# strasdat/ScaViSLAM

Hardware: AMD Instinct MI355X
Metric: stereo frames/sec + DWO Schur ms @ 50 KF / 20k pts (higher is better)
Workload: dtype u8/int32 (FAST, ZNSSD), f32+f64 (dense tracking), f64 (Schur); 1 GPU

## Files before the change

include/scavislam_hip.h:

```cpp
#ifndef SCAVISLAM_HIP_H
#define SCAVISLAM_HIP_H

#include <stddef.h>
#include <stdint.h>

#ifdef __cplusplus
extern "C" {
#endif

#define SVS_API_VERSION 9
int svs_api_version(void);

enum {
  SVS_OK = 0,
  SVS_ERR_INVALID = 1,
  SVS_ERR_HIP = 2,
  SVS_ERR_NO_DEVICE = 3,
  SVS_ERR_CAPACITY = 4,
  SVS_ERR_UNSUPPORTED = 5,
  SVS_ERR_BUSY = 6
};

#define SVS_NUM_PYR_LEVELS 3
#define SVS_MAX_CELLS 64

typedef struct { double f, cx, cy, b; int32_t w, h; } svs_cam;

typedef struct {
  int32_t gx, gy, cell_w, cell_h;
  int32_t min_inner, min_outer, max_inner, max_outer;
  int32_t fast_min, fast_max;
  int32_t thr[SVS_MAX_CELLS];
} svs_fastgrid;

typedef struct {
  double xyz_anchor[3];
  double anchor_obs_pyr[3];
  int32_t anchor_level, kf_index, point_id, pad_;
} svs_candidate_point;

typedef struct {
  double T_anchor_from_w[12];
  const uint8_t *pyr[3];
  int32_t stride[3];
  int32_t pad_;
} svs_keyframe;

enum { SVS_MATCH_OK = 0, SVS_MATCH_NO_ANCHOR, SVS_MATCH_BORDER, SVS_MATCH_DEPTH,
       SVS_MATCH_TEXTURE, SVS_MATCH_NONE, SVS_MATCH_NO_DISP,
       SVS_MATCH_SKIPPED  };

typedef struct {
  int32_t status, u, v, znssd;
  double obs[3];
  double xyz_actkey[3];
} svs_match_result;

typedef struct {
  double H[21];
  double b[6];
  double chi2;
  int64_t n_valid;
} svs_dense_sums;

typedef struct {
  double obs[3];
  double info[3];
  int32_t point, pose, anchor, pad_;
} svs_ba_edge;

typedef struct {
  double T_21[12];
  double info[36];
  int32_t pose1, pose2;
} svs_ba_constraint;

typedef struct {
  int32_t num_iters;
  int32_t use_robust;
  double huber_delta;
  double lambda_init;
  int32_t max_trials;
  int32_t self_edge_mode;
} svs_ba_params;

typedef struct {
  int32_t iterations, trials, accepted, terminated;
  double chi2_init, chi2_final, lambda_final;
} svs_ba_stats;

typedef struct svs_ctx svs_ctx;
int svs_ctx_create(int device, void *hip_stream, svs_ctx **out);
int svs_ctx_destroy(svs_ctx *ctx);
int svs_ctx_sync(svs_ctx *ctx);
int svs_ctx_set_option(svs_ctx *ctx, const char *name, int value);
int svs_ctx_get_stat(svs_ctx *ctx, const char *name, long long *out);
void *svs_ctx_stream(svs_ctx *ctx);
const char *svs_last_error(svs_ctx *ctx);
int svs_malloc(svs_ctx *ctx, size_t bytes, void **d_ptr);
int svs_free(svs_ctx *ctx, void *d_ptr);
int svs_memcpy_h2d(svs_ctx *ctx, void *d_dst, const void *h_src, size_t bytes);
int svs_memcpy_d2h(svs_ctx *ctx, void *h_dst, const void *d_src, size_t bytes);
int svs_timer_start(svs_ctx *ctx);
int svs_timer_stop_ms(svs_ctx *ctx, float *ms);

int svs_pyr_down_u8(svs_ctx *ctx, const uint8_t *d_src, int w, int h, int sstride, size_t s_bstride,
                    uint8_t *d_dst, int dstride, size_t d_bstride, int batch);
int svs_convert_sobel_f32(svs_ctx *ctx, const uint8_t *d_src, int w, int h, int sstride,
                          size_t s_bstride, float *d_img, float *d_dx, float *d_dy, int fstride,
                          size_t f_bstride, int batch);

typedef struct {
  int32_t prefilter_cap;
  int32_t sad_window;
  int32_t min_disparity;
  int32_t num_disparities;
  int32_t texture_threshold;
  int32_t uniqueness_ratio;
  int32_t speckle_window;
  int32_t speckle_range;
  int32_t disp12_max_diff;
} svs_stereo_params;
typedef struct svs_stereo svs_stereo;
int svs_stereo_create(svs_ctx *ctx, int w, int h, int max_batch, const svs_stereo_params *prm, svs_stereo **out);
int svs_stereo_destroy(svs_stereo *s);
int svs_stereo_compute(svs_stereo *s, const uint8_t *d_left, int lstride, size_t l_bstride, const uint8_t *d_right,
                       int rstride, size_t r_bstride, float *d_disp, int dstride, size_t d_bstride, int n_batch);

typedef struct svs_fast svs_fast;
int svs_fast_create(svs_ctx *ctx, int n_levels, const int32_t *w, const int32_t *h,
                    const svs_fastgrid *grids, int batch, int corner_cap_per_level,
                    svs_fast **out);
int svs_fast_destroy(svs_fast *f);
int svs_fast_detect(svs_fast *f, const uint8_t *const *d_img, const int32_t *stride,
                    const size_t *bstride, int n_batch, int trials);
int svs_fast_download(svs_fast *f, int slot, int level, int16_t *h_xy, int cap, int32_t *h_n,
                      int32_t *h_cell_count, int32_t *h_emit_thr, int32_t *h_thr_state);
int svs_fast_set_thresholds(svs_fast *f, int slot, int level, const int32_t *h_thr);
int svs_fast_device_view(svs_fast *f, int level, const uint32_t **d_corner_bits, int32_t *row_stride_bytes, size_t *batch_stride_bytes,
                         int32_t *cell_column_bits, const int32_t **d_emit_thr, size_t *emit_bstride);

typedef struct {
  const svs_keyframe *d_kfs; int32_t n_kf;
  const svs_candidate_point *d_pts; int32_t n_pts;
  const double *d_T_cur_from_w;
  const double *d_T_w_from_actkey;
  const uint8_t *d_cur_pyr[3]; int32_t cur_stride[3]; size_t cur_bstride[3];
  const float *d_disp; int32_t disp_stride; size_t disp_bstride;
  svs_cam cam_vec[3];
  int32_t search_radius, thr_mean, thr_std;
  int32_t n_batch;
  size_t kf_bstride, pts_bstride, out_bstride;
} svs_match_args;
int svs_match(svs_ctx *ctx, const svs_match_args *a, svs_fast *f, svs_match_result *d_out);

typedef struct {
  int32_t robust_kernel;
  int32_t num_iter;
  double kernel_param;
  double initial_mu;
  double tau;
  int32_t min_obs;
  int32_t pad_;
} svs_pose_opt_params;
void svs_pose_opt_params_default(svs_pose_opt_params *p);
typedef struct {
  double initial_chi2, chi2, max_err;
  int32_t num_obs;
  int32_t status;
} svs_pose_opt_stats;
int svs_motion_only(svs_ctx *ctx, const svs_match_result *d_results, int n, size_t res_bstride, const svs_cam *cam,
                    const svs_pose_opt_params *prm, double *d_T_io, svs_pose_opt_stats *d_stats, int batch);

typedef struct {
  int32_t accepted;
  int32_t is_new;
  double uv_pyr[2];
  double curkey_uv_pyr[2];
} svs_gated_point;
typedef struct {
  int32_t num_points_grid2x2[4];
  int32_t num_points_grid3x3[9];
  int32_t num_matched_points[3];
  int32_t num_track_points;
  int32_t num_obs;
  int32_t pad_[2];
  double sum_track_length;
} svs_point_stats;
int svs_process_matched_points(svs_ctx *ctx, const svs_match_result *d_results, const svs_candidate_point *d_pts, int n,
                               size_t res_bstride, size_t pts_bstride, int n_new_records, const svs_cam *cam,
                               const double *d_T, float max_reproj_error, svs_gated_point *d_gated, size_t gated_bstride,
                               svs_point_stats *d_stats, int batch);

int svs_pointcloud_cpu_sem(svs_ctx *ctx, const float *d_disp, int disp_stride, size_t disp_bstride,
                           const svs_cam *cam, int level, const double *d_T_cur_from_actkey,
                           float *d_cloud, size_t cloud_bstride, int batch);
int svs_dense_pass_cpu_sem(svs_ctx *ctx, const float *d_cloud, size_t cloud_bstride,
                           const uint8_t *d_prev_u8, int pstride, size_t p_bstride,
                           const float *d_cur, const float *d_dx, const float *d_dy, int fstride,
                           size_t f_bstride, const svs_cam *cam, const double *d_T, int do_jac,
                           svs_dense_sums *d_out, int batch);
typedef struct {
  int32_t level;
  int32_t accepted;
  float chi2, new_chi2;
} svs_dense_lm_record;
typedef struct {
  const float *d_cloud[3]; size_t cloud_bstride[3];
  const uint8_t *d_prev_u8[3]; int32_t pstride[3]; size_t p_bstride[3];
  const float *d_cur[3]; const float *d_dx[3]; const float *d_dy[3];
  int32_t fstride[3]; size_t f_bstride[3];
  svs_cam cam_vec[3];
  const uint8_t *d_cur_u8[3]; int32_t c8stride[3]; size_t c8_bstride[3];
  double *d_T_jac_out;
  svs_dense_lm_record *d_record_out;
  int32_t record_cap;
  int32_t *d_n_record_out;
} svs_dense_track_args;
int svs_dense_track_cpu_sem(svs_ctx *ctx, const svs_dense_track_args *a, double *d_T_io,
                            int32_t *d_passes_out, int batch);
int svs_dense_seq_sum_f32(svs_ctx *ctx, const float *d_terms, int n, size_t bstride, int batch, int how, float *d_out, int32_t *d_fell_back);
int svs_dense_residual_image_cpu_sem(svs_ctx *ctx, const float *d_cloud, size_t cloud_bstride,
                                     const uint8_t *d_prev_u8, int pstride, size_t p_bstride,
                                     const float *d_cur, int fstride, size_t f_bstride,
                                     const uint8_t *d_cur_u8, int c8stride, size_t c8_bstride,
                                     const svs_cam *cam, const double *d_T, size_t T_bstride,
                                     float *d_res_img4, size_t res_bstride, int batch);
int svs_preprocess_gpu_sem(svs_ctx *ctx, const uint8_t *d_src, int w, int h, int sstride, size_t s_bstride,
                           float *const *d_img, float *const *d_dx, float *const *d_dy, const int32_t *fstride,
                           const size_t *f_bstride, int levels, int batch);
typedef struct {
  const float *d_cloud4[3]; int32_t stride_f4[3]; size_t cloud_bstride[3];
  const float *d_prev[3];
  const float *d_cur[3];
  const float *d_dx[3], *d_dy[3];
  int32_t stride_f[3]; size_t f_bstride[3];
  int32_t w[3], h[3];
  double f[3], cx[3], cy[3];
  double *d_T_jac_out;
  svs_dense_lm_record *d_record_out;
  int32_t record_cap;
  int32_t *d_n_record_out;
} svs_dense_track_full_args;
int svs_dense_track_full(svs_ctx *ctx, const svs_dense_track_full_args *a, double *d_T_io, int32_t *d_passes_out, int batch);
int svs_dense_pixel_terms_full(svs_ctx *ctx, const float *d_cloud4, int w, int h, int stride_f4, const float *d_prev,
                               const float *d_cur, const float *d_dx, const float *d_dy, int stride_f, float f, float cx,
                               float cy, const float *h_T34_colmajor, float *d_terms8);
int svs_dense_pass_full(svs_ctx *ctx, const float *d_cloud4, int w, int h, int stride_f4,
                        const float *d_prev, const float *d_cur, const float *d_dx,
                        const float *d_dy, int stride_f, float f, float cx, float cy,
                        const float *h_T34_colmajor, int do_jac, svs_dense_sums *d_out);
int svs_dense_residual_image_full(svs_ctx *ctx, const float *d_cloud4, int w, int h, int stride_f4,
                                  const float *d_prev, const float *d_cur, int stride_f, float f,
                                  float cx, float cy, const float *h_T34_colmajor, float *d_res_img4);
int svs_pointcloud_full(svs_ctx *ctx, const float *h_TQ_colmajor, const float *d_disp, int w, int h,
                        int stride_in, int stride_out, int factor, float *d_cloud4);
int svs_pointcloud_full_pose(svs_ctx *ctx, const double *d_T, const svs_cam *cam, const float *d_disp, int disp_stride, size_t disp_bstride,
                             int w, int h, int stride_out, size_t cloud_bstride, int factor, float *d_cloud4, int batch);

typedef struct {
  int32_t fast_trials;
  int32_t search_radius, thr_mean, thr_std;
  float max_reproj_error;
  int32_t use_block_matching;
  svs_pose_opt_params pose_opt;
  svs_stereo_params stereo;
  int32_t n_levels;
  int32_t num_max_points;
  int32_t min_matches;
  int32_t cuda_build;
} svs_frontend_params;
typedef struct {
  double T_cur_from_actkey[12];
  int32_t dense_passes;
  int32_t n_points;
  int32_t n_matched;
  int32_t tracking_ok;
  svs_pose_opt_stats pose_stats;
  svs_point_stats point_stats;
} svs_frame_result;
typedef struct svs_frontend svs_frontend;
int svs_frontend_create(svs_ctx *ctx, const svs_cam *cam, const svs_frontend_params *prm, int max_points, int max_keyframes, svs_frontend **out);
int svs_frontend_create_batch(svs_ctx *ctx, const svs_cam *cam, const svs_frontend_params *prm, int max_points, int max_keyframes, int n_streams,
                              svs_frontend **out);
int svs_frontend_destroy(svs_frontend *fe);
int svs_frontend_first_frame(svs_frontend *fe, const uint8_t *h_left, int lstride, const uint8_t *h_right, int rstride, const float *h_disp, int dstride);
int svs_frontend_keep_keyframe(svs_frontend *fe, int slot, const double *T_kf_from_w);
int svs_frontend_keep_keyframe_of(svs_frontend *fe, int stream, int slot, const double *T_kf_from_w);
int svs_frontend_keep_keyframes(svs_frontend *fe, int slot, const double *h_T_kf_from_w);
int svs_frontend_set_candidates(svs_frontend *fe, const svs_candidate_point *h_pts, int n, int n_new_records);
int svs_frontend_set_candidates_grouped(svs_frontend *fe, int stream, const svs_candidate_point *h_pts, int n, const int32_t *h_group_end, int n_groups);
int svs_frontend_set_candidates_all(svs_frontend *fe, const svs_candidate_point *h_pts, const int32_t *h_n, const int32_t *h_group_end, int n_groups);
int svs_frontend_process_frame(svs_frontend *fe, const uint8_t *h_left, int lstride, const uint8_t *h_right, int rstride, const float *h_disp,
                               int dstride, const double *T_cur_from_actkey, const double *T_actkey_from_w, svs_frame_result *out,
                               svs_match_result *h_matches, svs_gated_point *h_gated);
int svs_frontend_submit_frame(svs_frontend *fe, const uint8_t *h_left, int lstride, const uint8_t *h_right, int rstride, const float *h_disp, int dstride,
                              const double *T_cur_from_actkey, const double *T_actkey_from_w, int want_matches, int want_gated);
int svs_frontend_wait_frame(svs_frontend *fe, svs_frame_result *out, svs_match_result *h_matches, svs_gated_point *h_gated);
int svs_frontend_prefetch_frame(svs_frontend *fe, const uint8_t *h_left, int lstride, const uint8_t *h_right, int rstride, const float *h_disp, int dstride);
int svs_frontend_staging_view(svs_frontend *fe, uint8_t **h_left, uint8_t **h_right, float **h_disp);
typedef struct {
  const uint8_t *d_left; int32_t lstride; size_t l_bstride;
  const uint8_t *d_right; int32_t rstride; size_t r_bstride;
  const float *d_disp; int32_t dstride; size_t d_bstride;
  void *ready_event;
} svs_frames_dev;
int svs_frontend_input_view(svs_frontend *fe, uint8_t **d_left, int32_t *lstride, size_t *l_bstride, uint8_t **d_right, int32_t *rstride, size_t *r_bstride,
                            float **d_disp, int32_t *dstride, size_t *d_bstride);
int svs_frontend_first_frames(svs_frontend *fe, const svs_frames_dev *in);
int svs_frontend_process_frames(svs_frontend *fe, const svs_frames_dev *in, const double *h_T_cur_from_actkey, const double *h_T_actkey_from_w);
int svs_frontend_results(svs_frontend *fe, int stream, svs_frame_result *out, svs_match_result *h_matches, svs_gated_point *h_gated);
int svs_frontend_poses(svs_frontend *fe, double *h_T_cur_from_actkey, int32_t *h_tracking_ok);
#define SVS_FRONTEND_STAGES 8
int svs_frontend_set_timing(svs_frontend *fe, int on);
int svs_frontend_stage_times(svs_frontend *fe, float *ms);
int svs_frontend_dense_records(svs_frontend *fe, int stream, svs_dense_lm_record *h_rec, int cap, int32_t *n);
int svs_frontend_recompute_cloud(svs_frontend *fe, const double *T_cur_from_actkey);
int svs_frontend_device_view(svs_frontend *fe, int stream, const uint8_t **d_pyr_last, int32_t *stride, const float **d_disp, const float **d_cloud,
                             svs_fast **fast);

typedef struct {
  int32_t clearance;
  int32_t num_max_points;
  int32_t min_num_points;
  int32_t n_levels;
} svs_seed_params;
void svs_seed_params_default(svs_seed_params *p);
typedef struct {
  double T_newkey_from_cur[12];
  uint64_t seed;
  int32_t add_flags[9];
  int32_t n0[3];
  int32_t n_tree;
  int32_t kf_index, first_point_id;
  int32_t use_order;
  int32_t n_order[3];
  int32_t pad_;
} svs_seed_problem;
typedef struct {
  const int16_t *d_xy[3]; size_t xy_bstride[3]; int32_t xy_cap[3];
  const int32_t *d_n[3]; size_t n_bstride[3];
  const int32_t *d_cell_count[3]; size_t cell_bstride[3]; int32_t n_cells[3];
  const float *d_disp; int32_t disp_stride; size_t disp_bstride;
  svs_cam cam;
  const svs_seed_problem *d_prob;
  const double *d_tree_xy; const int32_t *d_tree_level; size_t tree_bstride;
  const int32_t *d_order[3]; size_t order_bstride[3];
  int32_t batch;
} svs_seed_args;
int svs_seed_points(svs_ctx *ctx, const svs_seed_args *a, const svs_seed_params *prm, svs_candidate_point *d_out, int cap, int32_t *d_n_new);
enum { SVS_SEED_FIRST = 0,
       SVS_SEED_MORE = 1 };
typedef struct {
  int32_t stream, mode;
  int32_t kf_index, first_point_id;
  double T_newkey_from_cur[12];
  uint64_t seed;
  const int32_t *h_order[3];
  int32_t n_order[3];
  int32_t pad_;
} svs_seed_request;
int svs_frontend_seed_keyframes(svs_frontend *fe, int n, const svs_seed_request *req, const svs_seed_params *prm, svs_candidate_point *h_out, int cap_per_request,
                                int32_t *h_n_new);

int svs_rectify_build_maps(const double *K, const double *dist, const double *R, const double *Knew, int w, int h, int16_t *map_xy, uint16_t *map_frac);
typedef struct svs_rectify svs_rectify;
int svs_rectify_create(svs_ctx *ctx, int w, int h, int max_batch, const int16_t *h_left_xy, const uint16_t *h_left_frac, const int16_t *h_right_xy,
                       const uint16_t *h_right_frac, svs_rectify **out);
int svs_rectify_destroy(svs_rectify *r);
typedef struct {
  const uint8_t *d_left; int32_t lstride; size_t l_bstride;
  int32_t left_channels;
  const uint8_t *d_right; int32_t rstride; size_t r_bstride;
  void *ready_event;
} svs_raw_frames_dev;
int svs_rectify_frames(svs_rectify *r, const svs_raw_frames_dev *raw, uint8_t *d_left_out, int lstride, size_t l_bstride, uint8_t *d_right_out, int rstride,
                       size_t r_bstride, int n_batch);
int svs_depth_to_disp(svs_ctx *ctx, const svs_cam *cam, const uint16_t *d_depth16, int stride, size_t bstride, float *d_disp, int dstride, size_t d_bstride,
                      int n_batch);

typedef struct svs_loop svs_loop;
int svs_loop_create(svs_ctx *ctx, const svs_cam *cam, int desc_dim, int max_desc, int max_places, int max_hyp, int max_checks, svs_loop **out);
int svs_loop_destroy(svs_loop *l);
int svs_loop_set_place(svs_loop *l, int slot, int n, const float *h_desc, const double *h_uvu, const double *h_xyz);
typedef struct {
  int32_t query_slot, train_slot;
  int32_t n_hyp;
  double pixel_thr;
  uint64_t seed;
  const int32_t *h_samples;
} svs_loop_check;
typedef struct {
  int32_t n_matches;
  int32_t n_inliers;
  int32_t best_hyp;
  int32_t n_invalid_hyp;
  double T_query_from_train[12];
} svs_loop_result;
int svs_loop_check_batch(svs_loop *l, int n_checks, const svs_loop_check *checks, svs_loop_result *h_results, int32_t *h_train_idx, float *h_distance,
                         uint8_t *h_inlier, int32_t *h_samples_out, int32_t *h_hyp_inliers);
int svs_loop_set_timing(svs_loop *l, int on);
int svs_loop_stage_times(svs_loop *l, float *ms);

#define SVS_LOOP_MAX_WORDS 1048576
int svs_loop_set_vocabulary(svs_loop *l, int n_words, const float *h_words);
typedef struct {
  int32_t slot;
  int32_t do_loop_detection;
  const int32_t *h_exclude;
  int32_t n_exclude;
  float radius;
  float min_score;
} svs_loop_location;
typedef struct {
  int32_t number_of_words;
  int32_t n_scored;
  int32_t best_slot;
  float best_score;
  int32_t candidate;
} svs_loop_location_result;
int svs_loop_add_locations(svs_loop *l, int n, const svs_loop_location *locs, svs_loop_location_result *h_results, int32_t *h_word, float *h_word_d2,
                           float *h_scores);
int svs_loop_index_stage_times(svs_loop *l, float *ms);

#define SVS_VOCAB_MAX_POINTS 2097152
typedef struct {
  int32_t n_words;
  int32_t iterations;
  uint64_t seed;
  const float *h_init;
  int32_t drop_empty;
} svs_vocab_params;
typedef struct {
  int32_t n_words_out, n_seeded, iterations_run, converged, n_empty;
  uint64_t inertia_q28;
} svs_vocab_result;
void svs_vocab_params_default(svs_vocab_params *p);
int svs_vocab_train(svs_ctx *ctx, int desc_dim, int n, const float *h_desc, const svs_vocab_params *prm, float *h_words, svs_vocab_result *h_res,
                    int32_t *h_seed_index, int32_t *h_assign, float *h_assign_d2, int32_t *h_count, int32_t *h_changed);
int svs_vocab_stage_times(svs_ctx *ctx, float *ms);

typedef struct svs_surf svs_surf;
typedef struct {
  float hessian_threshold;
  int32_t n_octaves, n_octave_layers;
  int32_t require_disparity;
} svs_surf_params;
typedef struct { float x, y, size, angle, response; int32_t octave, laplacian, pad_; } svs_surf_keypoint;
#define SVS_SURF_STAGES 6
void svs_surf_params_default(svs_surf_params *p);
int svs_surf_create(svs_ctx *ctx, const svs_cam *cam, int w, int h, int max_batch, int max_keypoints, const svs_surf_params *prm, svs_surf **out);
int svs_surf_destroy(svs_surf *s);
int svs_surf_extract(svs_surf *s, const uint8_t *d_img, int stride, size_t bstride, const float *d_disp, int dstride, size_t d_bstride, int n_batch,
                     int32_t *h_count, int32_t *h_overflow, svs_surf_keypoint *h_kp, double *h_uvu, float *h_desc);
int svs_loop_set_place_from_surf(svs_loop *l, int slot, svs_surf *s, int image_index);
int svs_surf_set_timing(svs_surf *s, int on);
int svs_surf_stage_times(svs_surf *s, float *ms);

enum { SVS_REG_LOCAL = 0, SVS_REG_LOOP = 1 };
enum { SVS_REG_OK = 0, SVS_REG_FEW_CANDIDATES = 1, SVS_REG_FEW_MATCHES_PASS1 = 2, SVS_REG_FEW_MATCHES_PASS2 = 3, SVS_REG_NOT_COVISIBLE = 4 };
enum { SVS_REG_KF_IN_WINDOW = 1,
       SVS_REG_KF_DIRECT_NEIGHBOR = 2 };
typedef struct {
  int32_t covis_thr;
  int32_t search_radius[2];
  int32_t thr_mean, thr_std;
  int32_t num_iter[2];
  int32_t pad_;
  double reproj_thr;
  double kernel_param;
} svs_reg_params;
void svs_reg_params_default(svs_reg_params *p);
typedef struct {
  int32_t mode;
  int32_t n_kf, n_src;
  int32_t root_kf;
  const float *d_root_disp;
  int32_t root_disp_stride, pad_;
  int32_t fast_thr[SVS_NUM_PYR_LEVELS][SVS_MAX_CELLS];
  double T_root_from_world[12];
  const svs_keyframe *h_kfs;
  const uint8_t *h_kf_flags;
  const svs_candidate_point *h_src;
  const int32_t *h_obs_begin;
  const int32_t *h_obs_kf;
} svs_reg_request;
typedef struct {
  int32_t status;
  int32_t n_candidates, n_obs_pass1, n_obs_pass2, n_accepted;
  int32_t n_qualified;
  double T_newroot_from_oldroot[12];
  double T_pass1[12];
  svs_pose_opt_stats stats_pass1, stats_pass2;
} svs_reg_result;
typedef struct {
  int32_t strength;
  int32_t n_u_hi, n_u_lo, n_v_hi, n_v_lo;
  int32_t qualifies;
  int32_t in_vertex_table;
  int32_t pad_;
} svs_reg_kf_stats;
typedef struct svs_reg svs_reg;
int svs_reg_create(svs_ctx *ctx, const svs_cam *cam, int max_requests, int max_points, int max_keyframes, int max_observers, svs_reg **out);
int svs_reg_destroy(svs_reg *reg);
int svs_reg_register_batch(svs_reg *reg, int n_requests, const svs_reg_request *req, const svs_reg_params *prm, svs_reg_result *h_res, int32_t *h_cand_src,
                           svs_match_result *h_matches, int32_t *h_status_pass1, int32_t *h_accepted, svs_reg_kf_stats *h_kf_stats,
                           svs_match_result *h_matches_pass1);
#define SVS_REG_STAGES 7
int svs_reg_set_timing(svs_reg *reg, int on);
int svs_reg_stage_times(svs_reg *reg, float *ms);

typedef struct { char bytes[128]; } svs_unique_id;
typedef struct svs_comm svs_comm;
int svs_comm_get_unique_id(svs_ctx *ctx, svs_unique_id *out);
int svs_comm_create(svs_ctx *ctx, const svs_unique_id *id, int rank, int world, svs_comm **out);
int svs_comm_destroy(svs_comm *c);
int svs_comm_allreduce_f64(svs_comm *c, void *d_buf, size_t count);
int svs_comm_stats(svs_comm *c, int32_t *rank, int32_t *world, uint64_t *n_calls, uint64_t *n_doubles);
typedef struct { char bytes[64]; } svs_ipc_handle;
int svs_comm_create_p2p(svs_ctx *ctx, int rank, int world, size_t capacity_doubles, svs_comm **out, svs_ipc_handle *h_mine);
int svs_comm_connect_p2p(svs_comm *c, const svs_ipc_handle *h_all);
int svs_comm_transport(svs_comm *c, int32_t *kind, uint32_t *timeouts);

typedef struct svs_ba svs_ba;
typedef int (*svs_allreduce_fn)(void *d_buf, size_t count, void *user);

int svs_ba_create(svs_ctx *ctx, svs_ba **out);
int svs_ba_destroy(svs_ba *ba);
int svs_ba_set_problem(svs_ba *ba, int P, const double *h_poses, int L, const double *h_psi,
                       int E, const svs_ba_edge *h_edges, int C, const svs_ba_constraint *h_cons,
                       const svs_cam *cam, const svs_ba_params *prm, int add_pose_terms);
int svs_ba_window_update(svs_ba *ba, int P, const int32_t *h_pose_ids, const double *h_poses, int L, const int32_t *h_point_ids,
                         const double *h_psi, const int32_t *h_anchor_pose_ids, int n_new, const svs_ba_edge *h_new_obs, int C,
                         const svs_ba_constraint *h_cons, const svs_cam *cam, const svs_ba_params *prm);
int svs_ba_window_reset(svs_ba *ba);
int svs_ba_window_forget_keyframes(svs_ba *ba, const int32_t *h_pose_ids, int n);
int svs_ba_optimize(svs_ba *ba, svs_allreduce_fn allreduce, void *user, svs_ba_stats *stats);
int svs_ba_optimize_batch(svs_ba *const *bas, int n, svs_ba_stats *stats);
int svs_ba_get_state(svs_ba *ba, double *h_poses, double *h_psi);
int svs_ba_set_comm(svs_ba *ba, svs_comm *comm);
int svs_ba_set_option(svs_ba *ba, const char *name, int value);
int svs_ba_reset_state(svs_ba *ba, const double *h_poses, const double *h_psi);
int svs_ba_reduced_system(svs_ba *ba, double lambda, double *h_Hred ,
                          double *h_bred , double *h_chi2);
int svs_ba_schur_layout(svs_ba *ba, int32_t *waves_per_workgroup, int32_t *big_pool);
int svs_ba_trial(svs_ba *ba, double lambda, const double *h_xp, double *h_poses_trial, double *h_psi_trial, double *h_chi2_trial,
                 double *h_scale_l);
int svs_ba_info(svs_ba *ba, int32_t *solve_kind, int32_t *envelope_rows, int32_t *n_chunks, int32_t *n_wide);
int svs_ba_order_info(svs_ba *ba, int32_t *ordered, int32_t *envelope_rows_caller_order, int32_t *h_perm);
int svs_ba_set_timing(svs_ba *ba, int on);
int svs_ba_kernel_times(svs_ba *ba, float *reduce_ms, float *solve_ms, float *backsub_ms,
                        int32_t *n_reduce_launches);
int svs_ba_graph_stats(svs_ba *ba, int64_t *launches, int64_t *captures);

#ifdef __cplusplus
}
#endif
#endif
```

scavislam_amd/capi.py:

```python
import ctypes as C
import os
import weakref

from .ctypes_types import BaParams, BaStats, Cam, FastGrid, LoopCheck, LoopLocation, LoopLocationResult, LoopResult, PoseOptParams, PoseOptStats, RegParams, RegRequest, RegResult, SeedArgs, SeedParams, SeedRequest, StereoParams, SurfParams, VocabParams, VocabResult

_HERE = os.path.dirname(os.path.abspath(__file__))
LIB_PATH = os.environ.get("SVS_LIB_PATH") or os.path.join(_HERE, "libscavislam_hip.so")
_LIB = None

ALLREDUCE_FN = C.CFUNCTYPE(C.c_int, C.c_void_p, C.c_size_t, C.c_void_p)


class SvsError(RuntimeError):
    pass


class DenseTrackArgs(C.Structure):
    _fields_ = [("d_cloud", C.c_void_p * 3), ("cloud_bstride", C.c_size_t * 3),
                ("d_prev_u8", C.c_void_p * 3), ("pstride", C.c_int32 * 3), ("p_bstride", C.c_size_t * 3),
                ("d_cur", C.c_void_p * 3), ("d_dx", C.c_void_p * 3), ("d_dy", C.c_void_p * 3),
                ("fstride", C.c_int32 * 3), ("f_bstride", C.c_size_t * 3), ("cam_vec", Cam * 3),
                ("d_cur_u8", C.c_void_p * 3), ("c8stride", C.c_int32 * 3), ("c8_bstride", C.c_size_t * 3),
                ("d_T_jac_out", C.c_void_p), ("d_record_out", C.c_void_p), ("record_cap", C.c_int32), ("d_n_record_out", C.c_void_p)]


class DenseTrackFullArgs(C.Structure):
    _fields_ = [("d_cloud4", C.c_void_p * 3), ("stride_f4", C.c_int32 * 3), ("cloud_bstride", C.c_size_t * 3),
                ("d_prev", C.c_void_p * 3), ("d_cur", C.c_void_p * 3), ("d_dx", C.c_void_p * 3), ("d_dy", C.c_void_p * 3),
                ("stride_f", C.c_int32 * 3), ("f_bstride", C.c_size_t * 3),
                ("w", C.c_int32 * 3), ("h", C.c_int32 * 3),
                ("f", C.c_double * 3), ("cx", C.c_double * 3), ("cy", C.c_double * 3),
                ("d_T_jac_out", C.c_void_p), ("d_record_out", C.c_void_p), ("record_cap", C.c_int32),
                ("d_n_record_out", C.c_void_p)]


class FrontendParams(C.Structure):
    _fields_ = [("fast_trials", C.c_int32), ("search_radius", C.c_int32), ("thr_mean", C.c_int32), ("thr_std", C.c_int32),
                ("max_reproj_error", C.c_float), ("use_block_matching", C.c_int32), ("pose_opt", PoseOptParams), ("stereo", StereoParams),
                ("n_levels", C.c_int32), ("num_max_points", C.c_int32), ("min_matches", C.c_int32), ("cuda_build", C.c_int32)]

    @classmethod
    def reference(cls, use_block_matching=False, cuda_build=False, n_levels=3, search_radius=None, thr_mean=22, thr_std=10, num_max_points=300):
        if search_radius is None:
            search_radius = 4 if cuda_build else 8
        return cls(6, search_radius, thr_mean, thr_std, 2.0, int(use_block_matching), PoseOptParams.reference(), StereoParams.reference(),
                   n_levels, num_max_points, 20, int(cuda_build))


class FramesDev(C.Structure):
    _fields_ = [("d_left", C.c_void_p), ("lstride", C.c_int32), ("l_bstride", C.c_size_t),
                ("d_right", C.c_void_p), ("rstride", C.c_int32), ("r_bstride", C.c_size_t),
                ("d_disp", C.c_void_p), ("dstride", C.c_int32), ("d_bstride", C.c_size_t),
                ("ready_event", C.c_void_p)]


class PointStatsC(C.Structure):
    _fields_ = [("num_points_grid2x2", C.c_int32 * 4), ("num_points_grid3x3", C.c_int32 * 9), ("num_matched_points", C.c_int32 * 3),
                ("num_track_points", C.c_int32), ("num_obs", C.c_int32), ("pad_", C.c_int32 * 2), ("sum_track_length", C.c_double)]


class FrameResult(C.Structure):
    _fields_ = [("T_cur_from_actkey", C.c_double * 12), ("dense_passes", C.c_int32), ("n_points", C.c_int32), ("n_matched", C.c_int32),
                ("tracking_ok", C.c_int32), ("pose_stats", PoseOptStats), ("point_stats", PointStatsC)]


class MatchArgs(C.Structure):
    _fields_ = [("d_kfs", C.c_void_p), ("n_kf", C.c_int32),
                ("d_pts", C.c_void_p), ("n_pts", C.c_int32),
                ("d_T_cur_from_w", C.c_void_p), ("d_T_w_from_actkey", C.c_void_p),
                ("d_cur_pyr", C.c_void_p * 3), ("cur_stride", C.c_int32 * 3), ("cur_bstride", C.c_size_t * 3),
                ("d_disp", C.c_void_p), ("disp_stride", C.c_int32), ("disp_bstride", C.c_size_t),
                ("cam_vec", Cam * 3),
                ("search_radius", C.c_int32), ("thr_mean", C.c_int32), ("thr_std", C.c_int32),
                ("n_batch", C.c_int32),
                ("kf_bstride", C.c_size_t), ("pts_bstride", C.c_size_t), ("out_bstride", C.c_size_t)]


class RawFramesDev(C.Structure):
    _fields_ = [("d_left", C.c_void_p), ("lstride", C.c_int32), ("l_bstride", C.c_size_t), ("left_channels", C.c_int32),
                ("d_right", C.c_void_p), ("rstride", C.c_int32), ("r_bstride", C.c_size_t),
                ("ready_event", C.c_void_p)]


_SIGS = {
    "svs_ctx_create": [C.c_int, C.c_void_p, C.POINTER(C.c_void_p)],
    "svs_ctx_destroy": [C.c_void_p],
    "svs_ctx_sync": [C.c_void_p],
    "svs_ctx_set_option": [C.c_void_p, C.c_char_p, C.c_int],
    "svs_ctx_get_stat": [C.c_void_p, C.c_char_p, C.POINTER(C.c_longlong)],
    "svs_malloc": [C.c_void_p, C.c_size_t, C.POINTER(C.c_void_p)],
    "svs_free": [C.c_void_p, C.c_void_p],
    "svs_memcpy_h2d": [C.c_void_p, C.c_void_p, C.c_void_p, C.c_size_t],
    "svs_memcpy_d2h": [C.c_void_p, C.c_void_p, C.c_void_p, C.c_size_t],
    "svs_timer_start": [C.c_void_p],
    "svs_timer_stop_ms": [C.c_void_p, C.POINTER(C.c_float)],
    "svs_pyr_down_u8": [C.c_void_p, C.c_void_p, C.c_int, C.c_int, C.c_int, C.c_size_t, C.c_void_p, C.c_int,
                        C.c_size_t, C.c_int],
    "svs_convert_sobel_f32": [C.c_void_p, C.c_void_p, C.c_int, C.c_int, C.c_int, C.c_size_t, C.c_void_p,
                              C.c_void_p, C.c_void_p, C.c_int, C.c_size_t, C.c_int],
    "svs_fast_create": [C.c_void_p, C.c_int, C.POINTER(C.c_int32), C.POINTER(C.c_int32), C.POINTER(FastGrid),
                        C.c_int, C.c_int, C.POINTER(C.c_void_p)],
    "svs_fast_destroy": [C.c_void_p],
    "svs_fast_detect": [C.c_void_p, C.POINTER(C.c_void_p), C.POINTER(C.c_int32), C.POINTER(C.c_size_t),
                        C.c_int, C.c_int],
    "svs_fast_download": [C.c_void_p, C.c_int, C.c_int, C.c_void_p, C.c_int, C.POINTER(C.c_int32),
                          C.c_void_p, C.c_void_p, C.c_void_p],
    "svs_fast_set_thresholds": [C.c_void_p, C.c_int, C.c_int, C.c_void_p],
    "svs_fast_device_view": [C.c_void_p, C.c_int, C.POINTER(C.c_void_p), C.POINTER(C.c_int32), C.POINTER(C.c_size_t), C.POINTER(C.c_int32),
                             C.POINTER(C.c_void_p), C.POINTER(C.c_size_t)],
    "svs_match": [C.c_void_p, C.POINTER(MatchArgs), C.c_void_p, C.c_void_p],
    "svs_pointcloud_cpu_sem": [C.c_void_p, C.c_void_p, C.c_int, C.c_size_t, C.POINTER(Cam), C.c_int,
                               C.c_void_p, C.c_void_p, C.c_size_t, C.c_int],
    "svs_dense_pass_cpu_sem": [C.c_void_p, C.c_void_p, C.c_size_t, C.c_void_p, C.c_int, C.c_size_t,
                               C.c_void_p, C.c_void_p, C.c_void_p, C.c_int, C.c_size_t, C.POINTER(Cam),
                               C.c_void_p, C.c_int, C.c_void_p, C.c_int],
    "svs_dense_seq_sum_f32": [C.c_void_p, C.c_void_p, C.c_int, C.c_size_t, C.c_int, C.c_int, C.c_void_p, C.c_void_p],
    "svs_dense_track_cpu_sem": [C.c_void_p, C.POINTER(DenseTrackArgs), C.c_void_p, C.c_void_p, C.c_int],
    "svs_dense_residual_image_cpu_sem": [C.c_void_p, C.c_void_p, C.c_size_t, C.c_void_p, C.c_int, C.c_size_t,
                                         C.c_void_p, C.c_int, C.c_size_t, C.c_void_p, C.c_int, C.c_size_t,
                                         C.POINTER(Cam), C.c_void_p, C.c_size_t, C.c_void_p, C.c_size_t, C.c_int],
    "svs_dense_residual_image_full": [C.c_void_p, C.c_void_p, C.c_int, C.c_int, C.c_int, C.c_void_p, C.c_void_p,
                                      C.c_int, C.c_float, C.c_float, C.c_float, C.c_void_p, C.c_void_p],
    "svs_preprocess_gpu_sem": [C.c_void_p, C.c_void_p, C.c_int, C.c_int, C.c_int, C.c_size_t, C.POINTER(C.c_void_p), C.POINTER(C.c_void_p),
                               C.POINTER(C.c_void_p), C.POINTER(C.c_int32), C.POINTER(C.c_size_t), C.c_int, C.c_int],
    "svs_dense_track_full": [C.c_void_p, C.POINTER(DenseTrackFullArgs), C.c_void_p, C.c_void_p, C.c_int],
    "svs_dense_pixel_terms_full": [C.c_void_p, C.c_void_p, C.c_int, C.c_int, C.c_int, C.c_void_p, C.c_void_p, C.c_void_p, C.c_void_p,
                                   C.c_int, C.c_float, C.c_float, C.c_float, C.c_void_p, C.c_void_p],
    "svs_dense_pass_full": [C.c_void_p, C.c_void_p, C.c_int, C.c_int, C.c_int, C.c_void_p, C.c_void_p,
                            C.c_void_p, C.c_void_p, C.c_int, C.c_float, C.c_float, C.c_float, C.c_void_p,
                            C.c_int, C.c_void_p],
    "svs_pointcloud_full": [C.c_void_p, C.c_void_p, C.c_void_p, C.c_int, C.c_int, C.c_int, C.c_int, C.c_int,
                            C.c_void_p],
    "svs_motion_only": [C.c_void_p, C.c_void_p, C.c_int, C.c_size_t, C.POINTER(Cam), C.POINTER(PoseOptParams), C.c_void_p, C.c_void_p,
                        C.c_int],
    "svs_process_matched_points": [C.c_void_p, C.c_void_p, C.c_void_p, C.c_int, C.c_size_t, C.c_size_t, C.c_int, C.POINTER(Cam),
                                   C.c_void_p, C.c_float, C.c_void_p, C.c_size_t, C.c_void_p, C.c_int],
    "svs_stereo_create": [C.c_void_p, C.c_int, C.c_int, C.c_int, C.POINTER(StereoParams), C.POINTER(C.c_void_p)],
    "svs_stereo_destroy": [C.c_void_p],
    "svs_stereo_compute": [C.c_void_p, C.c_void_p, C.c_int, C.c_size_t, C.c_void_p, C.c_int, C.c_size_t, C.c_void_p, C.c_int,
                           C.c_size_t, C.c_int],
    "svs_frontend_create": [C.c_void_p, C.POINTER(Cam), C.POINTER(FrontendParams), C.c_int, C.c_int, C.POINTER(C.c_void_p)],
    "svs_frontend_create_batch": [C.c_void_p, C.POINTER(Cam), C.POINTER(FrontendParams), C.c_int, C.c_int, C.c_int, C.POINTER(C.c_void_p)],
    "svs_frontend_keep_keyframe_of": [C.c_void_p, C.c_int, C.c_int, C.c_void_p],
    "svs_frontend_set_candidates_grouped": [C.c_void_p, C.c_int, C.c_void_p, C.c_int, C.c_void_p, C.c_int],
    "svs_frontend_keep_keyframes": [C.c_void_p, C.c_int, C.c_void_p],
    "svs_frontend_set_candidates_all": [C.c_void_p, C.c_void_p, C.c_void_p, C.c_void_p, C.c_int],
    "svs_frontend_submit_frame": [C.c_void_p, C.c_void_p, C.c_int, C.c_void_p, C.c_int, C.c_void_p, C.c_int, C.c_void_p, C.c_void_p, C.c_int, C.c_int],
    "svs_frontend_wait_frame": [C.c_void_p, C.POINTER(FrameResult), C.c_void_p, C.c_void_p],
    "svs_frontend_prefetch_frame": [C.c_void_p, C.c_void_p, C.c_int, C.c_void_p, C.c_int, C.c_void_p, C.c_int],
    "svs_frontend_staging_view": [C.c_void_p, C.POINTER(C.c_void_p), C.POINTER(C.c_void_p), C.POINTER(C.c_void_p)],
    "svs_frontend_input_view": [C.c_void_p, C.POINTER(C.c_void_p), C.POINTER(C.c_int32), C.POINTER(C.c_size_t), C.POINTER(C.c_void_p), C.POINTER(C.c_int32),
                                C.POINTER(C.c_size_t), C.POINTER(C.c_void_p), C.POINTER(C.c_int32), C.POINTER(C.c_size_t)],
    "svs_frontend_first_frames": [C.c_void_p, C.POINTER(FramesDev)],
    "svs_frontend_process_frames": [C.c_void_p, C.POINTER(FramesDev), C.c_void_p, C.c_void_p],
    "svs_frontend_results": [C.c_void_p, C.c_int, C.POINTER(FrameResult), C.c_void_p, C.c_void_p],
    "svs_frontend_poses": [C.c_void_p, C.c_void_p, C.c_void_p],
    "svs_frontend_set_timing": [C.c_void_p, C.c_int],
    "svs_frontend_stage_times": [C.c_void_p, C.c_void_p],
    "svs_frontend_dense_records": [C.c_void_p, C.c_int, C.c_void_p, C.c_int, C.POINTER(C.c_int32)],
    "svs_pointcloud_full_pose": [C.c_void_p, C.c_void_p, C.POINTER(Cam), C.c_void_p, C.c_int, C.c_size_t, C.c_int, C.c_int, C.c_int, C.c_size_t, C.c_int,
                                 C.c_void_p, C.c_int],
    "svs_frontend_destroy": [C.c_void_p],
    "svs_frontend_first_frame": [C.c_void_p, C.c_void_p, C.c_int, C.c_void_p, C.c_int, C.c_void_p, C.c_int],
    "svs_frontend_keep_keyframe": [C.c_void_p, C.c_int, C.c_void_p],
    "svs_frontend_set_candidates": [C.c_void_p, C.c_void_p, C.c_int, C.c_int],
    "svs_frontend_process_frame": [C.c_void_p, C.c_void_p, C.c_int, C.c_void_p, C.c_int, C.c_void_p, C.c_int, C.c_void_p, C.c_void_p,
                                   C.POINTER(FrameResult), C.c_void_p, C.c_void_p],
    "svs_frontend_recompute_cloud": [C.c_void_p, C.c_void_p],
    "svs_frontend_device_view": [C.c_void_p, C.c_int, C.c_void_p, C.c_void_p, C.c_void_p, C.c_void_p, C.c_void_p],
    "svs_rectify_build_maps": [C.c_void_p, C.c_void_p, C.c_void_p, C.c_void_p, C.c_int, C.c_int, C.c_void_p, C.c_void_p],
    "svs_rectify_create": [C.c_void_p, C.c_int, C.c_int, C.c_int, C.c_void_p, C.c_void_p, C.c_void_p, C.c_void_p, C.POINTER(C.c_void_p)],
    "svs_rectify_destroy": [C.c_void_p],
    "svs_rectify_frames": [C.c_void_p, C.POINTER(RawFramesDev), C.c_void_p, C.c_int, C.c_size_t, C.c_void_p, C.c_int, C.c_size_t, C.c_int],
    "svs_depth_to_disp": [C.c_void_p, C.POINTER(Cam), C.c_void_p, C.c_int, C.c_size_t, C.c_void_p, C.c_int, C.c_size_t, C.c_int],
    "svs_seed_points": [C.c_void_p, C.POINTER(SeedArgs), C.POINTER(SeedParams), C.c_void_p, C.c_int, C.c_void_p],
    "svs_frontend_seed_keyframes": [C.c_void_p, C.c_int, C.POINTER(SeedRequest), C.POINTER(SeedParams), C.c_void_p, C.c_int, C.c_void_p],
    "svs_loop_create": [C.c_void_p, C.POINTER(Cam), C.c_int, C.c_int, C.c_int, C.c_int, C.c_int, C.POINTER(C.c_void_p)],
    "svs_loop_destroy": [C.c_void_p],
    "svs_loop_set_place": [C.c_void_p, C.c_int, C.c_int, C.c_void_p, C.c_void_p, C.c_void_p],
    "svs_loop_check_batch": [C.c_void_p, C.c_int, C.POINTER(LoopCheck), C.POINTER(LoopResult), C.c_void_p, C.c_void_p, C.c_void_p, C.c_void_p, C.c_void_p],
    "svs_loop_set_timing": [C.c_void_p, C.c_int],
    "svs_loop_stage_times": [C.c_void_p, C.c_void_p],
    "svs_loop_set_vocabulary": [C.c_void_p, C.c_int, C.c_void_p],
    "svs_loop_add_locations": [C.c_void_p, C.c_int, C.POINTER(LoopLocation), C.POINTER(LoopLocationResult), C.c_void_p, C.c_void_p, C.c_void_p],
    "svs_loop_index_stage_times": [C.c_void_p, C.c_void_p],
    "svs_vocab_train": [C.c_void_p, C.c_int, C.c_int, C.c_void_p, C.POINTER(VocabParams), C.c_void_p, C.POINTER(VocabResult), C.c_void_p, C.c_void_p, C.c_void_p,
                        C.c_void_p, C.c_void_p],
    "svs_vocab_stage_times": [C.c_void_p, C.c_void_p],
    "svs_surf_create": [C.c_void_p, C.POINTER(Cam), C.c_int, C.c_int, C.c_int, C.c_int, C.POINTER(SurfParams), C.POINTER(C.c_void_p)],
    "svs_surf_destroy": [C.c_void_p],
    "svs_surf_extract": [C.c_void_p, C.c_void_p, C.c_int, C.c_size_t, C.c_void_p, C.c_int, C.c_size_t, C.c_int, C.c_void_p, C.c_void_p, C.c_void_p, C.c_void_p,
                         C.c_void_p],
    "svs_loop_set_place_from_surf": [C.c_void_p, C.c_int, C.c_void_p, C.c_int],
    "svs_surf_set_timing": [C.c_void_p, C.c_int],
    "svs_surf_stage_times": [C.c_void_p, C.c_void_p],
    "svs_reg_create": [C.c_void_p, C.POINTER(Cam), C.c_int, C.c_int, C.c_int, C.c_int, C.POINTER(C.c_void_p)],
    "svs_reg_destroy": [C.c_void_p],
    "svs_reg_register_batch": [C.c_void_p, C.c_int, C.POINTER(RegRequest), C.POINTER(RegParams), C.POINTER(RegResult), C.c_void_p, C.c_void_p, C.c_void_p, C.c_void_p,
                               C.c_void_p, C.c_void_p],
    "svs_reg_set_timing": [C.c_void_p, C.c_int],
    "svs_reg_stage_times": [C.c_void_p, C.c_void_p],
    "svs_ba_create": [C.c_void_p, C.POINTER(C.c_void_p)],
    "svs_ba_destroy": [C.c_void_p],
    "svs_ba_set_problem": [C.c_void_p, C.c_int, C.c_void_p, C.c_int, C.c_void_p, C.c_int, C.c_void_p,
                           C.c_int, C.c_void_p, C.POINTER(Cam), C.POINTER(BaParams), C.c_int],
    "svs_ba_window_update": [C.c_void_p, C.c_int, C.c_void_p, C.c_void_p, C.c_int, C.c_void_p, C.c_void_p, C.c_void_p, C.c_int, C.c_void_p, C.c_int,
                             C.c_void_p, C.POINTER(Cam), C.POINTER(BaParams)],
    "svs_ba_window_reset": [C.c_void_p],
    "svs_ba_window_forget_keyframes": [C.c_void_p, C.c_void_p, C.c_int],
    "svs_ba_optimize": [C.c_void_p, C.c_void_p, C.c_void_p, C.POINTER(BaStats)],
    "svs_ba_optimize_batch": [C.POINTER(C.c_void_p), C.c_int, C.POINTER(BaStats)],
    "svs_ba_get_state": [C.c_void_p, C.c_void_p, C.c_void_p],
    "svs_ba_reset_state": [C.c_void_p, C.c_void_p, C.c_void_p],
    "svs_ba_reduced_system": [C.c_void_p, C.c_double, C.c_void_p, C.c_void_p, C.c_void_p],
    "svs_ba_info": [C.c_void_p, C.POINTER(C.c_int32), C.POINTER(C.c_int32), C.POINTER(C.c_int32), C.POINTER(C.c_int32)],
    "svs_ba_schur_layout": [C.c_void_p, C.POINTER(C.c_int32), C.POINTER(C.c_int32)],
    "svs_ba_trial": [C.c_void_p, C.c_double, C.c_void_p, C.c_void_p, C.c_void_p, C.c_void_p, C.c_void_p],
    "svs_ba_order_info": [C.c_void_p, C.POINTER(C.c_int32), C.POINTER(C.c_int32), C.c_void_p],
    "svs_ba_set_timing": [C.c_void_p, C.c_int],
    "svs_ba_set_option": [C.c_void_p, C.c_char_p, C.c_int],
    "svs_ba_set_comm": [C.c_void_p, C.c_void_p],
    "svs_comm_get_unique_id": [C.c_void_p, C.c_void_p],
    "svs_comm_create": [C.c_void_p, C.c_void_p, C.c_int, C.c_int, C.POINTER(C.c_void_p)],
    "svs_comm_destroy": [C.c_void_p],
    "svs_comm_allreduce_f64": [C.c_void_p, C.c_void_p, C.c_size_t],
    "svs_comm_stats": [C.c_void_p, C.POINTER(C.c_int32), C.POINTER(C.c_int32), C.POINTER(C.c_uint64), C.POINTER(C.c_uint64)],
    "svs_comm_create_p2p": [C.c_void_p, C.c_int, C.c_int, C.c_size_t, C.POINTER(C.c_void_p), C.c_void_p],
    "svs_comm_connect_p2p": [C.c_void_p, C.c_void_p],
    "svs_comm_transport": [C.c_void_p, C.POINTER(C.c_int32), C.POINTER(C.c_uint32)],
    "svs_ba_kernel_times": [C.c_void_p, C.POINTER(C.c_float), C.POINTER(C.c_float), C.POINTER(C.c_float),
                            C.POINTER(C.c_int32)],
    "svs_ba_graph_stats": [C.c_void_p, C.POINTER(C.c_int64), C.POINTER(C.c_int64)],
}
EXPORTS = sorted(list(_SIGS) + ["svs_ctx_stream", "svs_last_error", "svs_api_version", "svs_pose_opt_params_default", "svs_seed_params_default", "svs_reg_params_default", "svs_vocab_params_default", "svs_surf_params_default"])
API_VERSION = 9


def load():
    global _LIB
    if _LIB is None:
        if not os.path.exists(LIB_PATH):
            raise SvsError(f"{LIB_PATH} not built: run `python -c 'import __graft_entry__ as g; g.build()'` "
                           "(there is no CPU fallback)")
        import torch
        lib = C.CDLL(LIB_PATH)
        for name, args in _SIGS.items():
            fn = getattr(lib, name)
            fn.argtypes = args
            fn.restype = C.c_int
        lib.svs_ctx_stream.argtypes = [C.c_void_p]
        lib.svs_ctx_stream.restype = C.c_void_p
        lib.svs_last_error.argtypes = [C.c_void_p]
        lib.svs_last_error.restype = C.c_char_p
        lib.svs_api_version.argtypes = []
        lib.svs_api_version.restype = C.c_int
        lib.svs_pose_opt_params_default.argtypes = [C.c_void_p]
        lib.svs_pose_opt_params_default.restype = None
        lib.svs_seed_params_default.argtypes = [C.c_void_p]
        lib.svs_seed_params_default.restype = None
        lib.svs_reg_params_default.argtypes = [C.c_void_p]
        lib.svs_reg_params_default.restype = None
        lib.svs_vocab_params_default.argtypes = [C.c_void_p]
        lib.svs_vocab_params_default.restype = None
        lib.svs_surf_params_default.argtypes = [C.c_void_p]
        lib.svs_surf_params_default.restype = None
        if lib.svs_api_version() != API_VERSION:
            raise SvsError(f"{LIB_PATH} was built with SVS_API_VERSION {lib.svs_api_version()}, this binding expects {API_VERSION}: rebuild (__graft_entry__.build())")
        _LIB = lib
    return _LIB


class Context:

    def __init__(self, device=0, stream_ptr=None):
        self.lib = load()
        h = C.c_void_p()
        rc = self.lib.svs_ctx_create(int(device), C.c_void_p(stream_ptr) if stream_ptr else None, C.byref(h))
        if rc:
            raise SvsError(f"svs_ctx_create failed with status {rc} (no gfx950 device visible?)")
        self.h = h
        self.device = device
        self.children = weakref.WeakSet()

    def check(self, rc):
        if rc:
            raise SvsError(f"status {rc}: {self.lib.svs_last_error(self.h).decode(errors='replace')}")

    def call(self, name, *args):
        self.check(getattr(self.lib, name)(self.h, *args))

    def sync(self):
        self.check(self.lib.svs_ctx_sync(self.h))

    def set_option(self, name, value):
        self.call("svs_ctx_set_option", name.encode(), int(value))

    def get_stat(self, name):
        v = C.c_longlong(0)
        self.call("svs_ctx_get_stat", name.encode(), C.byref(v))
        return int(v.value)

    def timer_start(self):
        self.check(self.lib.svs_timer_start(self.h))

    def timer_stop_ms(self):
        ms = C.c_float()
        self.check(self.lib.svs_timer_stop_ms(self.h, C.byref(ms)))
        return ms.value

    def close(self):
        if self.h:
            for ch in list(self.children):
                ch.close()
            self.lib.svs_ctx_destroy(self.h)
            self.h = None

    def __del__(self):
        try:
            self.close()
        except Exception:
            pass


def torch_context(device=0):
    import torch
    torch.cuda.set_device(device)
    s = torch.cuda.Stream(device=device)
    return Context(device, s.cuda_stream), s
```

scavislam_amd/csrc/dense.hip:

```cpp
#include "common.h"
#include "lm6.h"
#include "seqsum.h"
#include <algorithm>
#include <climits>

namespace {

constexpr int NSUM = 28;

struct Acc {
  double v[NSUM];
  int n;
  __device__ __forceinline__ void zero() {
#pragma unroll
    for (int i = 0; i < NSUM; ++i) v[i] = 0;
    n = 0;
  }
};

template <class P>
__device__ __forceinline__ float interp32f(P m, int stride, float u, float v) {
  float x = floorf(u), y = floorf(v);
  float sx = u - x, sy = v - y;
  float wx0 = 1 - sx, wx1 = sx, wy0 = 1 - sy, wy1 = sy;
  int xi = (int)x, yi = (int)y;
  const P p = m + (unsigned)(yi * stride + xi);
  float v00 = p[0], v10 = p[1], v01 = p[stride], v11 = p[stride + 1];
  return (wx0 * wy0) * v00 + (wx0 * wy1) * v01 + (wx1 * wy0) * v10 + (wx1 * wy1) * v11;
}

struct LevelArgs {
  const float *cloud; const uint8_t *prev; const float *cur, *dx, *dy;
  int pstride, fstride;
  svs_cam cam;
  const uint8_t *cur8;
  int c8stride;
};

#define SVS_AS1 __attribute__((address_space(1)))
typedef float svs_f4 __attribute__((ext_vector_type(4)));
struct LevelArgsG {
  const SVS_AS1 float *cloud; const SVS_AS1 uint8_t *prev; const SVS_AS1 float *cur, *dx, *dy;
  int pstride, fstride;
  svs_cam cam;
  const SVS_AS1 uint8_t *cur8;
  int c8stride;
};
__device__ __forceinline__ float4 load_f4(const float *p) { return *reinterpret_cast<const float4 *>(p); }
__device__ __forceinline__ float4 load_f4(const SVS_AS1 float *p) { const svs_f4 v = *(const SVS_AS1 svs_f4 *)p; return make_float4(v.x, v.y, v.z, v.w); }
__device__ __forceinline__ uint32_t load_u32_unaligned(const uint8_t *p) { uint32_t w; __builtin_memcpy(&w, p, 4); return w; }
__device__ __forceinline__ uint32_t load_u32_unaligned(const SVS_AS1 uint8_t *p) {
  typedef uint32_t u32_unaligned __attribute__((aligned(1)));
  return *(const SVS_AS1 u32_unaligned *)p;
}

struct TapRows { uint32_t w[4]; };
constexpr bool TRK_TAPS_ASM = true;
template <bool ASM, class P>
__device__ __forceinline__ void taps_u8_issue(P img, int stride, float u, float v, TapRows &t) {
  const int xi = (int)floorf(u), yi = (int)floorf(v);
  const unsigned o0 = __umul24(yi - 1, stride) + (unsigned)(xi - 1);
  __builtin_amdgcn_sched_barrier(0);
  if constexpr (ASM) {
    const unsigned long long bv = (unsigned long long)img;
    const unsigned long long b0 = ((unsigned long long)(unsigned)__builtin_amdgcn_readfirstlane((int)(bv >> 32)) << 32) | (unsigned)__builtin_amdgcn_readfirstlane((int)bv);
    const unsigned long long rs = (unsigned long long)(unsigned)__builtin_amdgcn_readfirstlane(stride);
    asm("global_load_dword %0, %4, %5\n\t"
        "global_load_dword %1, %4, %6\n\t"
        "global_load_dword %2, %4, %7\n\t"
        "global_load_dword %3, %4, %8"
        : "=&v"(t.w[0]), "=&v"(t.w[1]), "=&v"(t.w[2]), "=&v"(t.w[3])
        : "v"(o0), "s"(b0), "s"(b0 + rs), "s"(b0 + 2 * rs), "s"(b0 + 3 * rs));
  } else {
#pragma unroll
    for (int r = 0; r < 4; ++r) t.w[r] = load_u32_unaligned(img + (o0 + (unsigned)(r * stride)));
  }
  __builtin_amdgcn_sched_barrier(0);
}
template <bool ASM>
__device__ __forceinline__ void taps_u8_wait(TapRows &t) {
  __builtin_amdgcn_sched_barrier(0);
  if constexpr (ASM) {
    asm("s_waitcnt vmcnt(0)" : "+v"(t.w[0]), "+v"(t.w[1]), "+v"(t.w[2]), "+v"(t.w[3]));
    __builtin_amdgcn_sched_barrier(0);
  }
}
__device__ __forceinline__ void taps_u8_finish(const TapRows &t, float u, float v, float &ic, float &gx, float &gy) {
  const float sc = (float)(1. / 255.);
  const float x = floorf(u), y = floorf(v);
  const float sx = u - x, sy = v - y;
  const float wx0 = 1 - sx, wx1 = sx, wy0 = 1 - sy, wy1 = sy;
  float f[4][4];
#pragma unroll
  for (int r = 0; r < 4; ++r)
#pragma unroll
    for (int c = 0; c < 4; ++c) f[r][c] = (float)((t.w[r] >> (8 * c)) & 0xff) * sc;
  const float w00 = wx0 * wy0, w01 = wx0 * wy1, w10 = wx1 * wy0, w11 = wx1 * wy1;
  ic = w00 * f[1][1] + w01 * f[2][1] + w10 * f[1][2] + w11 * f[2][2];
  gx = w00 * (f[1][2] - f[1][0]) + w01 * (f[2][2] - f[2][0]) + w10 * (f[1][3] - f[1][1]) + w11 * (f[2][3] - f[2][1]);
  gy = w00 * (f[2][1] - f[0][1]) + w01 * (f[3][1] - f[1][1]) + w10 * (f[2][2] - f[0][2]) + w11 * (f[3][2] - f[1][2]);
}
template <class P>
__device__ __forceinline__ void taps_u8(P img, int stride, float u, float v, float &ic, float &gx, float &gy) {
  TapRows t;
  taps_u8_issue<false>(img, stride, u, v, t);
  taps_u8_finish(t, u, v, ic, gx, gy);
}

struct SampleIn { float4 c4; uint8_t prev; };
template <class LA>
__device__ __forceinline__ SampleIn sample_load(const LA &L, int u, int v, int cw, bool in_range) {
  SampleIn s;
  s.c4 = in_range ? load_f4(L.cloud + 4u * (__umul24(v, cw) + (unsigned)u)) : make_float4(0.f, 0.f, 1.f, -1.f);
  s.prev = L.prev[__umul24((in_range ? v : 0) * 4, L.pstride) + (unsigned)((in_range ? u : 0) * 4)];
  return s;
}
__device__ __forceinline__ double rcp_rn(double b) {
  double r = __builtin_amdgcn_rcp(b);
  double e = __builtin_fma(-b, r, 1.0);
  r = __builtin_fma(e, r, r);
  e = __builtin_fma(-b, r, 1.0);
  return __builtin_fma(e, r, r);
}
__device__ __forceinline__ double div_rn(double a, double b, double r) {
  const double q = a * r;
  return __builtin_fma(__builtin_fma(-q, b, a), r, q);
}

template <bool JAC, bool U8SRC = false, int TM = 0, class LA = LevelArgs>
__device__ __forceinline__ void sample_cpu_sem(const LA &L, const double *T, const SampleIn &in, bool in_range, Acc &a,
                                               const float *ip_lut = nullptr, float *term_out = nullptr) {
  const float4 c4 = in.c4;
  bool ok = in_range && (c4.w > 0);
  const double xp0 = c4.x, xp1 = c4.y, xp2 = c4.z;
  const double x = T[0] * xp0 + T[1] * xp1 + T[2] * xp2 + T[3];
  const double y = T[4] * xp0 + T[5] * xp1 + T[6] * xp2 + T[7];
  const double z = T[8] * xp0 + T[9] * xp1 + T[10] * xp2 + T[11];
  const double rz = rcp_rn(z);
  float uvx = (float)(L.cam.f * div_rn(x, z, rz) + L.cam.cx);
  float uvy = (float)(L.cam.f * div_rn(y, z, rz) + L.cam.cy);
  ok = ok && (fabsf(uvx) < 1e9f && fabsf(uvy) < 1e9f);
  const int ui = ok ? (int)uvx : 0, vi = ok ? (int)uvy : 0;
  ok = ok && (ui >= 2 && vi >= 2 && ui < L.cam.w - 2 && vi < L.cam.h - 2);
  if (!ok) { uvx = 2.f; uvy = 2.f; }
  const float ip = ip_lut ? ip_lut[in.prev] : (float)((1. / 255.) * in.prev);
  TapRows taps;
  if constexpr (U8SRC) taps_u8_issue<TRK_TAPS_ASM>(L.cur8, L.c8stride, uvx, uvy, taps);
  const double zs = ok ? z : 1.0, xs = ok ? x : 0.0, ys = ok ? y : 0.0;
  const double f = L.cam.f, iz = ok ? rz : 1.0, iz2 = iz * iz, fx = f * iz, xz = xs * iz2 * f, yz = ys * iz2 * f;
  float ic, g8x = 0.f, g8y = 0.f;
  if constexpr (U8SRC) { taps_u8_wait<TRK_TAPS_ASM>(taps); taps_u8_finish(taps, uvx, uvy, ic, g8x, g8y); }
  else ic = interp32f(L.cur, L.fstride, uvx, uvy);
  const double r0[6] = {-fx, 0, xz, xz * ys, -__builtin_fma(xz, xs, f), ys * fx};
  const double r1[6] = {0, -fx, yz, __builtin_fma(yz, ys, f), -(yz * xs), -(xs * fx)};
  float res = ip - ic;
  res = fminf(fmaxf(res, -0.1f), 0.1f);
  if (!ok) res = 0.f;
  a.v[27] += (double)(res * res);
  if constexpr (TM != 0) *term_out = res * res;
  a.n += ok ? 1 : 0;
  if (JAC) {
    const float gx = ok ? (float)(0.5 * (U8SRC ? g8x : interp32f(L.dx, L.fstride, uvx, uvy))) : 0.f;
    const float gy = ok ? (float)(0.5 * (U8SRC ? g8y : interp32f(L.dy, L.fstride, uvx, uvy))) : 0.f;
    {
      double J[6];
      J[0] = gx * r0[0];
      J[1] = gy * r1[1];
#pragma unroll
      for (int k = 2; k < 6; ++k) J[k] = __builtin_fma(gx, r0[k], gy * r1[k]);
      int k = 0;
#pragma unroll
      for (int c = 0; c < 6; ++c)
#pragma unroll
        for (int r = 0; r <= c; ++r) { a.v[k] = __builtin_fma(J[r], J[c], a.v[k]); ++k; }
#pragma unroll
      for (int i = 0; i < 6; ++i) a.v[21 + i] = __builtin_fma(J[i], (double)res, a.v[21 + i]);
    }
  }
}

template <int NWAVES>
__device__ __forceinline__ void block_reduce(Acc &a, double (*s_part)[NSUM + 1], double *out_vals ) {
  const int lane = threadIdx.x & 63, wave = threadIdx.x >> 6;
  double x[32];
#pragma unroll
  for (int i = 0; i < NSUM; ++i) x[i] = a.v[i];
  x[NSUM] = (double)a.n;
#pragma unroll
  for (int i = NSUM + 1; i < 32; ++i) x[i] = 0.0;
#pragma unroll
  for (int step = 0; step < 5; ++step) {
    const int half = 16 >> step, bit = 1 << step;
    const bool up = (lane & bit) != 0;
#pragma unroll
    for (int k = 0; k < half; ++k) {
      const double send = up ? x[k] : x[k + half];
      const double keep = up ? x[k + half] : x[k];
      x[k] = keep + __shfl_xor(send, bit, 64);
    }
  }
  x[0] += __shfl_xor(x[0], 32, 64);
  const int idx = ((lane & 1) << 4) | ((lane & 2) << 2) | (lane & 4) | ((lane & 8) >> 2) | ((lane & 16) >> 4);
  if (lane < 32 && idx <= NSUM) s_part[wave][idx] = x[0];
  __syncthreads();
  if (threadIdx.x <= NSUM) {
    double s = 0;
    for (int w = 0; w < NWAVES; ++w) s += s_part[w][threadIdx.x];
    out_vals[threadIdx.x] = s;
  }
  __syncthreads();
}

template <bool JAC>
__global__ __launch_bounds__(256) void dense_pass_cpu_sem_kernel(LevelArgs L, size_t cloud_b, size_t prev_b, size_t f_b,
                                                                 const double *__restrict__ Tarr, double *__restrict__ partials) {
  __shared__ double s_part[4][NSUM + 1];
  __shared__ double s_out[NSUM + 1];
  const int slot = blockIdx.y;
  L.cloud += slot * cloud_b; L.prev += slot * prev_b; L.cur += slot * f_b; L.dx += slot * f_b; L.dy += slot * f_b;
  double T[12];
#pragma unroll
  for (int i = 0; i < 12; ++i) T[i] = Tarr[(size_t)slot * 12 + i];
  const int cw = L.cam.w / 4, ch = L.cam.h / 4, n = cw * ch;
  Acc a;
  a.zero();
  for (int i = blockIdx.x * 256 + threadIdx.x; i < n; i += gridDim.x * 256) sample_cpu_sem<JAC>(L, T, sample_load(L, i % cw, i / cw, cw, true), true, a);
  block_reduce<4>(a, s_part, s_out);
  if (threadIdx.x <= NSUM) partials[((size_t)slot * gridDim.x + blockIdx.x) * (NSUM + 1) + threadIdx.x] = s_out[threadIdx.x];
}

__global__ void dense_finalize_kernel(const double *__restrict__ partials, int nblocks, svs_dense_sums *__restrict__ out) {
  const int slot = blockIdx.x, t = threadIdx.x;
  if (t > NSUM) return;
  double s = 0;
  for (int b = 0; b < nblocks; ++b) s += partials[((size_t)slot * nblocks + b) * (NSUM + 1) + t];
  svs_dense_sums *o = &out[slot];
  if (t < 21) o->H[t] = s;
  else if (t < 27) o->b[t - 21] = s;
  else if (t == 27) o->chi2 = (double)(float)s;
  else o->n_valid = (long long)s;
}

struct TrackArgs {
  LevelArgs lv[3];
  size_t cloud_b[3], prev_b[3], f_b[3], c8_b[3];
  double *T_jac;
  svs_dense_lm_record *rec; int rec_cap; int32_t *n_rec;
};

constexpr int TRK_THREADS = 512;
constexpr int TRK_UNROLL = 1;
constexpr bool TRK_T_SCALAR = true;

template <bool JAC, bool U8SRC, int TM = 0, class LA = LevelArgs>
__device__ __forceinline__ void track_pass(const LA &L_in, const double *T_in, double (*s_part)[NSUM + 1], double *s_out, const float *ip_lut,
                                           int first, int nwg, float *t_buf = nullptr) {
  const LA L = L_in;
  const int cw = L.cam.w / 4, ch = L.cam.h / 4, n = cw * ch;
  double T[12];
#pragma unroll
  for (int i = 0; i < 12; ++i)
    T[i] = TRK_T_SCALAR ? __hiloint2double(__builtin_amdgcn_readfirstlane(__double2hiint(T_in[i])), __builtin_amdgcn_readfirstlane(__double2loint(T_in[i]))) : T_in[i];
  Acc a;
  a.zero();
  const int STEP = TRK_UNROLL * TRK_THREADS * nwg;
  const int su = STEP % cw, sv = STEP / cw;
  SampleIn nxt[TRK_UNROLL];
  int pu[TRK_UNROLL], pv[TRK_UNROLL];
#pragma unroll
  for (int q = 0; q < TRK_UNROLL; ++q) {
    const int j = first + q * TRK_THREADS * nwg;
    pu[q] = j % cw; pv[q] = j / cw;
    const bool in = pv[q] < ch;
    nxt[q] = sample_load(L, in ? pu[q] : 0, in ? pv[q] : 0, cw, in);
  }
  typedef __attribute__((address_space(1))) float *gptr_t;
  typedef __attribute__((address_space(1))) char *gptr_c;
  static_assert(TM == 0 || TRK_UNROLL == 1, "the deferred term store keeps one term per lane");
  float pend_t = 0.f;
  const gptr_c pend_base = (gptr_c)(gptr_t)t_buf - 4 * (long)STEP;
  bool pend = false;
  int i = first;
  auto flush = [&]() {
    const gptr_t pend_p = (gptr_t)(pend_base + 4u * (unsigned)i);
    if constexpr (TM == 1) { if (pend) *pend_p = pend_t; }
    if constexpr (TM == 2) { if (pend) __hip_atomic_store(pend_p, pend_t, __ATOMIC_RELAXED, __HIP_MEMORY_SCOPE_AGENT); }
  };
  for (; i < n; i += STEP) {
    if constexpr (TM != 0) { flush(); pend = t_buf != nullptr; }
    SampleIn cur[TRK_UNROLL];
#pragma unroll
    for (int q = 0; q < TRK_UNROLL; ++q) {
      cur[q] = nxt[q];
      pu[q] += su; pv[q] += sv;
      if (pu[q] >= cw) { pu[q] -= cw; ++pv[q]; }
      const bool in = pv[q] < ch;
      nxt[q] = sample_load(L, in ? pu[q] : 0, in ? pv[q] : 0, cw, in);
    }
#pragma unroll
    for (int q = 0; q < TRK_UNROLL; ++q) {
      if constexpr (TM != 0) sample_cpu_sem<JAC, U8SRC, TM, LA>(L, T, cur[q], true, a, ip_lut, &pend_t);
      else sample_cpu_sem<JAC, U8SRC, 0, LA>(L, T, cur[q], i + q * TRK_THREADS * nwg < n, a, ip_lut);
    }
  }
  if constexpr (TM != 0) flush();
  block_reduce<TRK_THREADS / 64>(a, s_part, s_out);
}

struct PassArgs { LevelArgs L; double T[12]; float *t_buf; int wg, nwg; };
__shared__ PassArgs g_pa;
__shared__ double g_s_part[TRK_THREADS / 64][NSUM + 1];
__shared__ double g_s_out[NSUM + 1];
__shared__ float g_iplut[256];
__device__ __forceinline__ int uni_i32(int v) { return __builtin_amdgcn_readfirstlane(v); }
__device__ __forceinline__ double uni_f64(double v) { return __hiloint2double(__builtin_amdgcn_readfirstlane(__double2hiint(v)), __builtin_amdgcn_readfirstlane(__double2loint(v))); }
template <class T>
__device__ __forceinline__ T *uni_ptr(T *p) {
  const unsigned long long u = (unsigned long long)p;
  const unsigned lo = __builtin_amdgcn_readfirstlane((unsigned)u), hi = __builtin_amdgcn_readfirstlane((unsigned)(u >> 32));
  return (T *)(((unsigned long long)hi << 32) | lo);
}
template <bool U8SRC, int TM>
__device__ __forceinline__ void track_pass_from_lds() {
  LevelArgsG L;
  L.cloud = (const SVS_AS1 float *)uni_ptr(g_pa.L.cloud); L.prev = (const SVS_AS1 uint8_t *)uni_ptr(g_pa.L.prev);
  L.cur = (const SVS_AS1 float *)uni_ptr(g_pa.L.cur); L.dx = (const SVS_AS1 float *)uni_ptr(g_pa.L.dx); L.dy = (const SVS_AS1 float *)uni_ptr(g_pa.L.dy);
  L.cur8 = (const SVS_AS1 uint8_t *)uni_ptr(g_pa.L.cur8);
  L.pstride = uni_i32(g_pa.L.pstride); L.fstride = uni_i32(g_pa.L.fstride); L.c8stride = uni_i32(g_pa.L.c8stride);
  L.cam.f = uni_f64(g_pa.L.cam.f); L.cam.cx = uni_f64(g_pa.L.cam.cx); L.cam.cy = uni_f64(g_pa.L.cam.cy); L.cam.b = 0;
  L.cam.w = uni_i32(g_pa.L.cam.w); L.cam.h = uni_i32(g_pa.L.cam.h);
  const int nwg = uni_i32(g_pa.nwg), first = uni_i32(g_pa.wg) * TRK_THREADS + (int)threadIdx.x;
  track_pass<true, U8SRC, TM, LevelArgsG>(L, g_pa.T, g_s_part, g_s_out, g_iplut, first, nwg, uni_ptr(g_pa.t_buf));
}

typedef const __attribute__((address_space(1))) float *svs_gptr_f32;
typedef const __attribute__((address_space(1))) svs_f4 *svs_gptr_f4;
template <bool COH, typename P>
__device__ __forceinline__ float seq_term_load(P p) {
  if constexpr (COH) return __hip_atomic_load(p, __ATOMIC_RELAXED, __HIP_MEMORY_SCOPE_AGENT); else return *p;
}
template <bool COH = false, typename P = const float *>
__device__ __forceinline__ float seq_sum_f32(P t, int n) {
  float acc = 0.f;
  const int lane = threadIdx.x & 63;
  for (int base = 0; base < n; base += 64) {
    const float v = base + lane < n ? seq_term_load<COH, P>(t + base + lane) : 0.f;
#pragma unroll
    for (int l = 0; l < 64; ++l) acc = acc + __builtin_bit_cast(float, __builtin_amdgcn_readlane(__builtin_bit_cast(int, v), l));
  }
  return acc;
}
__device__ __forceinline__ float seq_chi2_f32(const float *t, int n) {
  __shared__ float s_seq;
  __syncthreads();
  if (threadIdx.x < 64) { const float v = seq_sum_f32(t, n); if (threadIdx.x == 0) s_seq = v; }
  __syncthreads();
  return s_seq;
}

constexpr int SEQ_Q = TRK_THREADS >= 512 ? 10 : 13;
constexpr int SEQ_RUN_MAX = 4 * SEQ_Q;
constexpr int SEQ_STAGE_FLOATS = 48 * SEQ_RUN_MAX;
struct SeqShared {
  SvsSeqMap pref[TRK_THREADS];
  unsigned char eb[TRK_THREADS];
  short slot[TRK_THREADS];
  unsigned long long unsafe[TRK_THREADS / 64];
  double wave_P[TRK_THREADS / 64];
  int wave_c[TRK_THREADS / 64], wave_u[TRK_THREADS / 64];
  float stage[SEQ_STAGE_FLOATS];
  float result;
  int fell_back;
};
template <bool COH>
__device__ __forceinline__ void seq_load_run(svs_gptr_f32 p, int nq, svs_f4 (&v)[SEQ_Q]) {
  if constexpr (COH) {
    static_assert(SEQ_Q == 10 || SEQ_Q == 13, "the blocks below issue ten (+ three) loads");
    asm volatile("global_load_dwordx4 %0, %10, off sc1\n\t"
                 "global_load_dwordx4 %1, %10, off offset:16 sc1\n\t"
                 "global_load_dwordx4 %2, %10, off offset:32 sc1\n\t"
                 "global_load_dwordx4 %3, %10, off offset:48 sc1\n\t"
                 "global_load_dwordx4 %4, %10, off offset:64 sc1\n\t"
                 "global_load_dwordx4 %5, %10, off offset:80 sc1\n\t"
                 "global_load_dwordx4 %6, %10, off offset:96 sc1\n\t"
                 "global_load_dwordx4 %7, %10, off offset:112 sc1\n\t"
                 "global_load_dwordx4 %8, %10, off offset:128 sc1\n\t"
                 "global_load_dwordx4 %9, %10, off offset:144 sc1\n\t"
                 "s_waitcnt vmcnt(0)"
                 : "=&v"(v[0]), "=&v"(v[1]), "=&v"(v[2]), "=&v"(v[3]), "=&v"(v[4]), "=&v"(v[5]), "=&v"(v[6]), "=&v"(v[7]), "=&v"(v[8]), "=&v"(v[9])
                 : "v"(p)
                 : "memory");
    if constexpr (SEQ_Q == 13)
      asm volatile("global_load_dwordx4 %0, %3, off offset:160 sc1\n\t"
                   "global_load_dwordx4 %1, %3, off offset:176 sc1\n\t"
                   "global_load_dwordx4 %2, %3, off offset:192 sc1\n\t"
                   "s_waitcnt vmcnt(0)"
                   : "=&v"(v[SEQ_Q - 3]), "=&v"(v[SEQ_Q - 2]), "=&v"(v[SEQ_Q - 1])
                   : "v"(p)
                   : "memory");
  } else {
#pragma unroll
    for (int q = 0; q < SEQ_Q; ++q) v[q] = q < nq ? *reinterpret_cast<svs_gptr_f4>(p + 4 * q) : svs_f4{0.f, 0.f, 0.f, 0.f};
  }
}
__shared__ SeqShared g_seq_sh;
template <bool COH>
__device__ __noinline__ float exact_seq_sum_f32(const float *t_flat, int n) {
  SeqShared &sh = g_seq_sh;
  svs_gptr_f32 t = (svs_gptr_f32)t_flat;
  const int tid = threadIdx.x, lane = tid & 63, wave = tid >> 6;
  const int S = max(4, (div_up(n, TRK_THREADS) + 3) & ~3);
  if (S > SEQ_RUN_MAX) {
    __syncthreads();
    if (wave == 0) { const float v = seq_sum_f32<COH, svs_gptr_f32>(t, n); if (lane == 0) { sh.result = v; sh.fell_back = 1; } }
    __syncthreads();
    return sh.result;
  }
  const int nq = S / 4;
  const int j0 = min(n, tid * S), j1 = min(n, j0 + S);
  const bool empty = j0 >= j1;
  svs_f4 v[SEQ_Q];
  seq_load_run<COH>(t + (empty ? 0 : j0), nq, v);
  double ps = 0;
  int cnt = 0;
#pragma unroll
  for (int q = 0; q < SEQ_Q; ++q)
#pragma unroll
    for (int c = 0; c < 4; ++c) {
      if (!(q < nq && j0 + 4 * q + c < j1)) v[q][c] = 0.f;
      ps += (double)v[q][c];
      cnt += v[q][c] != 0.f ? 1 : 0;
    }
  double incl = ps;
  int cincl = cnt;
#pragma unroll
  for (int d = 1; d < 64; d <<= 1) {
    const double o = __shfl_up(incl, d, 64);
    const int oc = __shfl_up(cincl, d, 64);
    if (lane >= d) { incl += o; cincl += oc; }
  }
  __syncthreads();
  if (lane == 63) { sh.wave_P[wave] = incl; sh.wave_c[wave] = cincl; }
  __syncthreads();
  double base = 0;
  int cbase = 0;
  for (int w = 0; w < wave; ++w) { base += sh.wave_P[w]; cbase += sh.wave_c[w]; }
  const double excl = __shfl_up(incl, 1, 64);
  const int cexcl = __shfl_up(cincl, 1, 64);
  const double P_s = base + (lane ? excl : 0.0), P_e = P_s + ps;
  const int c_s = cbase + (lane ? cexcl : 0), c_e = c_s + cnt;
  int eb = 0;
  bool safe = empty || svs_seq_safe(P_s, P_e, c_s, c_e, &eb);
  sh.eb[tid] = (safe && !empty) ? (unsigned char)eb : (unsigned char)0;
  __syncthreads();
  if (safe && !empty && tid > 0) { const int pe = sh.eb[tid - 1]; if (pe != 0 && pe != eb) safe = false; }
  const unsigned long long um = __ballot(!safe);
  if (lane == 0) { sh.unsafe[wave] = um; sh.wave_u[wave] = __popcll(um); }
  __syncthreads();
  int ubase = 0;
  for (int w = 0; w < wave; ++w) ubase += sh.wave_u[w];
  const int uidx = ubase + __popcll(um & ((1ull << lane) - 1ull));
  const int slot = (!safe && (uidx + 1) * S <= SEQ_STAGE_FLOATS) ? uidx : -1;
  sh.slot[tid] = (short)slot;
  if (!safe) sh.eb[tid] = 0;
  SvsSeqMap m{0, 0};
  if (safe) {
#pragma unroll
    for (int q = 0; q < SEQ_Q; ++q)
#pragma unroll
      for (int c = 0; c < 4; ++c) svs_seq_add_term_fast(m, v[q][c], eb);
  } else if (slot >= 0) {
#pragma unroll
    for (int q = 0; q < SEQ_Q; ++q)
      if (q < nq) *reinterpret_cast<svs_f4 *>(&sh.stage[slot * S + 4 * q]) = v[q];
  }
  bool flag = !safe || lane == 0;
#pragma unroll
  for (int d = 1; d < 64; d <<= 1) {
    const int o0 = __shfl_up(m.d0, d, 64), o1 = __shfl_up(m.dd, d, 64), of = __shfl_up((int)flag, d, 64);
    if (lane >= d && !flag) { m = svs_seq_compose(SvsSeqMap{o0, o1}, m); flag = of != 0; }
  }
  sh.pref[tid] = m;
  __syncthreads();
  if (wave == 0) {
    float acc = 0.f;
    bool ok = true;
    const int nseg = div_up(n, S);
    for (int chunk = 0; chunk * 64 < nseg && ok; ++chunk) {
      const int limit = min(64, nseg - chunk * 64);
      const unsigned long long mask = sh.unsafe[chunk];
      const SvsSeqMap my = sh.pref[chunk * 64 + lane];
      const int my_eb = sh.eb[chunk * 64 + lane], my_sl = sh.slot[chunk * 64 + lane];
      auto run_terms = [&](int idx) {
        const int seg = chunk * 64 + idx, sj0 = seg * S, len = min(S, n - sj0), sl = __builtin_amdgcn_readlane(my_sl, idx);
        float x = sh.stage[(sl >= 0 && lane < len) ? sl * S + lane : 0];
        if (sl < 0) x = seq_term_load<COH, svs_gptr_f32>(t + sj0 + (lane < len ? lane : 0));
        return lane < len ? x : 0.f;
      };
      unsigned long long m = limit < 64 ? mask & ((1ull << limit) - 1ull) : mask;
      float x_next = m ? run_terms((int)__builtin_ctzll(m)) : 0.f;
      int pos = 0;
      while (ok) {
        const int nxt = m ? (int)__builtin_ctzll(m) : limit;
        if (nxt > pos) {
          const SvsSeqMap g{__builtin_amdgcn_readlane(my.d0, nxt - 1), __builtin_amdgcn_readlane(my.dd, nxt - 1)};
          ok = svs_seq_apply(&acc, g, __builtin_amdgcn_readlane(my_eb, nxt - 1));
        }
        if (nxt >= limit || !ok) break;
        m &= m - 1ull;
        const float x = x_next;
        if (m) x_next = run_terms((int)__builtin_ctzll(m));
#pragma unroll
        for (int l = 0; l < SEQ_RUN_MAX; ++l) acc = acc + __builtin_bit_cast(float, __builtin_amdgcn_readlane(__builtin_bit_cast(int, x), l));
        pos = nxt + 1;
      }
    }
    if (!ok) acc = seq_sum_f32<COH, svs_gptr_f32>(t, n);
    if (lane == 0) { sh.result = acc; if (!ok) sh.fell_back = 1; }
  }
  __syncthreads();
  return sh.result;
}

struct NearSums { float seq_old, seq_new; bool failed; };
template <bool COH>
__device__ __forceinline__ NearSums shared_near_sums(const float *t_old, const float *t_new, int n, int wg, int nwg, bool need_old, float seq_old_in, unsigned n_dec, unsigned n_old,
                                                     double *bc, unsigned *fail_word, unsigned &n_exact) {
  __shared__ unsigned long long s_words[2];
  __shared__ int s_nf;
  NearSums R{seq_old_in, 0.f, false};
  if (nwg <= 1) {
    if (need_old) { R.seq_old = exact_seq_sum_f32<COH>(t_old, n); ++n_exact; }
    R.seq_new = exact_seq_sum_f32<COH>(t_new, n); ++n_exact;
    return R;
  }
  unsigned long long *w_new = reinterpret_cast<unsigned long long *>(bc + 13), *w_old = reinterpret_cast<unsigned long long *>(bc + 15);
  if (wg == 0) {
    R.seq_new = exact_seq_sum_f32<COH>(t_new, n); ++n_exact;
    if (threadIdx.x == 0) __hip_atomic_store(w_new, ((unsigned long long)n_dec << 32) | (unsigned long long)__float_as_uint(R.seq_new), __ATOMIC_RELAXED, __HIP_MEMORY_SCOPE_AGENT);
  } else if (wg == 1 && need_old) {
    R.seq_old = exact_seq_sum_f32<COH>(t_old, n); ++n_exact;
    if (threadIdx.x == 0) __hip_atomic_store(w_old, ((unsigned long long)n_old << 32) | (unsigned long long)__float_as_uint(R.seq_old), __ATOMIC_RELAXED, __HIP_MEMORY_SCOPE_AGENT);
  }
  if (threadIdx.x == 0) {
    int nf = 0;
    auto wait_word = [&](const unsigned long long *w, unsigned want) {
      unsigned long long v = 0;
      long spin = 0;
      for (; spin < (1l << 24); ++spin) { v = __hip_atomic_load(w, __ATOMIC_RELAXED, __HIP_MEMORY_SCOPE_AGENT); if ((unsigned)(v >> 32) >= want) break; __builtin_amdgcn_s_sleep(1); }
      if (spin >= (1l << 24)) nf = 1;
      return v;
    };
    s_words[0] = wg == 0 ? 0ull : wait_word(w_new, n_dec);
    s_words[1] = (need_old && wg != 1) ? wait_word(w_old, n_old) : 0ull;
    if (nf) __hip_atomic_store(fail_word, 1u, __ATOMIC_RELAXED, __HIP_MEMORY_SCOPE_AGENT);
    s_nf = nf;
  }
  __syncthreads();
  if (wg != 0) R.seq_new = __uint_as_float((unsigned)s_words[0]);
  if (need_old && wg != 1) R.seq_old = __uint_as_float((unsigned)s_words[1]);
  R.failed = s_nf != 0;
  __syncthreads();
  return R;
}

#if defined(__HIP_DEVICE_COMPILE__) && !defined(__gfx950__) && !defined(__gfx942__)
#error "dense.hip: the relaxed-atomic + s_waitcnt vmcnt(0) hand-off is only valid on gfx950 / gfx942"
#endif
struct TrackMulti {
  double *part;
  unsigned *bar; int fail_off;
  double *bcast;
  const int *map;
  float *terms; size_t terms_b;
  unsigned *seq_stats;
  int terms_only;
  int *work16;
};

template <bool U8SRC>
__device__ __forceinline__ LevelArgs stream_level(const TrackArgs &A, int level, int slot) {
  LevelArgs L = A.lv[level];
  L.cloud += slot * A.cloud_b[level]; L.prev += slot * A.prev_b[level];
  if (U8SRC) L.cur8 += slot * A.c8_b[level];
  else { L.cur += slot * A.f_b[level]; L.dx += slot * A.f_b[level]; L.dy += slot * A.f_b[level]; }
  return L;
}
__device__ __forceinline__ void track_solve(const double (&sH)[27], const double (&sT)[12], double (&sTn)[12], double (&sx)[6]) {
  const int lane = threadIdx.x;
  double col[6], x[6], Tc[12], Tn[12];
#pragma unroll
  for (int r = 0; r < 6; ++r) {
    const int lo = r < lane ? r : lane, hi = r < lane ? lane : r;
    col[r] = lane < 6 ? sH[hi * (hi + 1) / 2 + lo] : (lane == 6 ? -sH[21 + r] : (r == 0 ? 1.0 : 0.0));
  }
  wave_solve6(col, x);
#pragma unroll
  for (int i = 0; i < 12; ++i) Tc[i] = sT[i];
  mo2_exp_mul(x, Tc, Tn);
  if (lane < 12) {
    double v = Tn[0];
#pragma unroll
    for (int i = 1; i < 12; ++i) v = lane == i ? Tn[i] : v;
    sTn[lane] = v;
  }
  if (lane < 6) {
    double v = x[0];
#pragma unroll
    for (int i = 1; i < 6; ++i) v = lane == i ? x[i] : v;
    sx[lane] = v;
  }
}
__device__ __forceinline__ void sum_workgroups(const TrackMulti &G, int slot, double *buf, int wg, int nwg, int &sweep, bool &s_failed) {
  if (threadIdx.x <= NSUM) __hip_atomic_store(buf + wg * 32 + threadIdx.x, g_s_out[threadIdx.x], __ATOMIC_RELAXED, __HIP_MEMORY_SCOPE_AGENT);
  asm volatile("s_waitcnt vmcnt(0)" ::: "memory");
  __syncthreads();
  ++sweep;
  if (threadIdx.x == 0) {
    __hip_atomic_fetch_add(G.bar + slot, 1u, __ATOMIC_RELAXED, __HIP_MEMORY_SCOPE_AGENT);
    const unsigned target = (unsigned)sweep * (unsigned)nwg;
    long spin = 0;
    for (; spin < (1l << 24) && __hip_atomic_load(G.bar + slot, __ATOMIC_RELAXED, __HIP_MEMORY_SCOPE_AGENT) < target; ++spin) __builtin_amdgcn_s_sleep(1);
    if (spin >= (1l << 24)) __hip_atomic_store(G.bar + G.fail_off + slot, 1u, __ATOMIC_RELAXED, __HIP_MEMORY_SCOPE_AGENT);
    s_failed = __hip_atomic_load(G.bar + G.fail_off + slot, __ATOMIC_RELAXED, __HIP_MEMORY_SCOPE_AGENT) != 0;
  }
  __syncthreads();
  if (threadIdx.x <= NSUM) {
    double acc = 0;
    for (int w = 0; w < nwg; ++w) acc += __hip_atomic_load(buf + w * 32 + threadIdx.x, __ATOMIC_RELAXED, __HIP_MEMORY_SCOPE_AGENT);
    g_s_out[threadIdx.x] = acc;
  }
  __syncthreads();
}
struct TrkVerdict { bool accept, failed; float chi2, new_chi2; };
template <bool MULTI>
__device__ __forceinline__ TrkVerdict track_accept(const TrackMulti &G, int slot, double S_old, double S_new, int nv_old, int nv_new, const float *tb0, int cur,
                                                   int n_lvl, bool counted, int wg, int nwg, float chi2, float &seq_old, bool &seq_old_ok,
                                                   unsigned &n_decisions, unsigned &n_old_sums, unsigned &n_exact) {
  TrkVerdict V{false, false, chi2, 0.f};
  const double gam = 1.0001 * (double)max(nv_old, nv_new) * 5.9604644775390625e-08 + 1e-12;
  const bool near = tb0 && !G.terms_only && !(fabs(S_old - S_new) > gam * (S_old + S_new));
  if (near) {
    if (counted) { ++n_decisions; if (!seq_old_ok) ++n_old_sums; }
    const NearSums ns = shared_near_sums<MULTI>(tb0 + (size_t)cur * G.terms_b, tb0 + (size_t)(cur ^ 1) * G.terms_b, n_lvl, wg, nwg, !seq_old_ok, seq_old, n_decisions, n_old_sums,
                                                MULTI ? G.bcast + (size_t)slot * 16 : nullptr, MULTI ? G.bar + G.fail_off + slot : nullptr, n_exact);
    if (ns.failed) { V.failed = true; return V; }
    seq_old = ns.seq_old;
    seq_old_ok = true;
    V.chi2 = seq_old; V.new_chi2 = ns.seq_new;
    V.accept = (double)V.chi2 - (double)V.new_chi2 > 0;
    if (V.accept) seq_old = ns.seq_new;
  } else {
    V.new_chi2 = (float)S_new;
    V.accept = S_old > S_new;
    if (V.accept) seq_old_ok = false;
  }
  return V;
}

template <bool U8SRC, bool MULTI, bool SEQ = false>
__global__ __launch_bounds__(TRK_THREADS, 2) void dense_track_cpu_sem_kernel(TrackArgs A, double *__restrict__ T_io, int *__restrict__ passes_out, TrackMulti G) {
  double (&s_out)[NSUM + 1] = g_s_out;
  float (&s_iplut)[256] = g_iplut;
  __shared__ double s_T[12], s_Tn[12], s_x[6], s_H[27], s_Tj[3][12];
  __shared__ bool s_failed;
  if (threadIdx.x == 0) { s_failed = false; if (!SEQ) g_seq_sh.fell_back = 0; }
  constexpr int TM = SEQ ? 1 : (MULTI ? 2 : 1);
  unsigned n_exact = 0, n_decisions = 0, n_old_sums = 0;
  const int slot = MULTI ? blockIdx.y : blockIdx.x, wg = MULTI ? blockIdx.x : 0;
  const int nwg = MULTI ? (int)gridDim.x : 1;
  const int first = wg * TRK_THREADS + threadIdx.x;
  int sweep = 0;
  auto all_workgroups = [&]() {
    if (!MULTI) return;
    const unsigned ep = (unsigned)(++sweep);
    unsigned long long *buf = reinterpret_cast<unsigned long long *>(G.part) + ((size_t)slot * 2 + (ep & 1u)) * (size_t)nwg * 64;
    bool timed_out = false;
    if (threadIdx.x < 2 * (NSUM + 1)) {
      const int k = threadIdx.x;
      const double mine = s_out[k >> 1];
      const unsigned my_half = (k & 1) ? (unsigned)__double2hiint(mine) : (unsigned)__double2loint(mine);
      __hip_atomic_store(buf + (size_t)wg * 64 + k, ((unsigned long long)ep << 32) | my_half, __ATOMIC_RELAXED, __HIP_MEMORY_SCOPE_AGENT);
      double acc = 0;
      long budget = 1l << 24;
      for (int w = 0; w < nwg; ++w) {
        unsigned h = my_half;
        if (w != wg) {
          unsigned long long v = __hip_atomic_load(buf + (size_t)w * 64 + k, __ATOMIC_RELAXED, __HIP_MEMORY_SCOPE_AGENT);
          while ((unsigned)(v >> 32) != ep && budget > 0) { __builtin_amdgcn_s_sleep(1); --budget; v = __hip_atomic_load(buf + (size_t)w * 64 + k, __ATOMIC_RELAXED, __HIP_MEMORY_SCOPE_AGENT); }
          if ((unsigned)(v >> 32) != ep) timed_out = true;
          h = (unsigned)v;
        }
        const unsigned other = (unsigned)__shfl_xor((int)h, 1, 64);
        acc += __hiloint2double((int)((k & 1) ? h : other), (int)((k & 1) ? other : h));
      }
      if (!(k & 1)) s_out[k >> 1] = acc;
    }
    if (__syncthreads_or(timed_out ? 1 : 0)) {
      if (threadIdx.x == 0) { __hip_atomic_store(G.bar + G.fail_off + slot, 1u, __ATOMIC_RELAXED, __HIP_MEMORY_SCOPE_AGENT); s_failed = true; }
      __syncthreads();
    }
  };
  if (threadIdx.x < 12) s_T[threadIdx.x] = T_io[(size_t)slot * 12 + threadIdx.x];
  for (int i = threadIdx.x; i < 256; i += TRK_THREADS) s_iplut[i] = (float)((1. / 255.) * i);
  __syncthreads();
  int passes = 0, n_rec = 0;
  bool failed = false;
  for (int level = 2; level >= 0; --level) {
    const bool solo = MULTI && level == 2;
    if (solo && wg != 0) {
      if (threadIdx.x == 0) {
        long spin = 0;
        for (; spin < (1l << 24) && __hip_atomic_load(reinterpret_cast<unsigned *>(G.bcast + (size_t)slot * 16 + 12), __ATOMIC_RELAXED, __HIP_MEMORY_SCOPE_AGENT) == 0u; ++spin)
          __builtin_amdgcn_s_sleep(2);
        if (spin >= (1l << 24)) s_failed = true;
      }
      __syncthreads();
      if (s_failed) { failed = true; break; }
      if (threadIdx.x < 12) s_T[threadIdx.x] = __hip_atomic_load(G.bcast + (size_t)slot * 16 + threadIdx.x, __ATOMIC_RELAXED, __HIP_MEMORY_SCOPE_AGENT);
      __syncthreads();
      continue;
    }
    const int lnwg = solo ? 1 : nwg;
    const LevelArgs L = stream_level<U8SRC>(A, level, slot);
    const int n_lvl = (L.cam.w / 4) * (L.cam.h / 4);
    __syncthreads();
    auto sweep_at = [&](const double *s_pose, float *t_buf) {
      track_pass<true, U8SRC, TM>(L, s_pose, g_s_part, g_s_out, g_iplut, solo ? (int)threadIdx.x : first, lnwg, t_buf);
    };
    float *tb[2];
    tb[0] = SEQ ? reinterpret_cast<float *>(G.part) + (size_t)slot * G.fail_off : (G.terms ? G.terms + (size_t)slot * 2 * G.terms_b : nullptr);
    tb[1] = SEQ ? tb[0] : (G.terms ? tb[0] + G.terms_b : nullptr);
    int cur = 0;
    sweep_at(s_T, tb[cur]);
    if (!solo) all_workgroups();
    if (MULTI && s_failed) { failed = true; break; }
    ++passes;
    float chi2;
    double S_old = s_out[27];
    int nv_old = (int)s_out[NSUM];
    float seq_old = 0.f;
    bool seq_old_ok = false;
    if constexpr (SEQ) chi2 = seq_chi2_f32(tb[0], n_lvl); else chi2 = (float)S_old;
    if (threadIdx.x < 27) s_H[threadIdx.x] = s_out[threadIdx.x];
    if (A.rec && wg == 0 && threadIdx.x == 0 && n_rec < A.rec_cap) A.rec[(size_t)slot * A.rec_cap + n_rec] = svs_dense_lm_record{level, 2, chi2, chi2};
    ++n_rec;
    __syncthreads();
    bool stop = false;
    for (int it = 0; it < 15 && !stop; ++it) {
      if (threadIdx.x >= 64 && threadIdx.x < 76) s_Tj[level][threadIdx.x - 64] = s_T[threadIdx.x - 64];
      if (threadIdx.x < 64) track_solve(s_H, s_T, s_Tn, s_x);
      __syncthreads();
      sweep_at(s_Tn, tb[cur ^ 1]);
      if (!solo) all_workgroups();
      if (MULTI && s_failed) { failed = true; break; }
      ++passes;
      float new_chi2;
      bool accept;
      const double S_new = s_out[27];
      const int nv_new = (int)s_out[NSUM];
      if constexpr (SEQ) {
        new_chi2 = seq_chi2_f32(tb[0], n_lvl);
        accept = (double)chi2 - (double)new_chi2 > 0;
      } else {
        const bool shared = MULTI && !solo;
        const TrkVerdict V = track_accept<MULTI>(G, slot, S_old, S_new, nv_old, nv_new, tb[0], cur, n_lvl, shared, shared ? wg : 0, shared ? nwg : 1,
                                                 chi2, seq_old, seq_old_ok, n_decisions, n_old_sums, n_exact);
        if (V.failed) { s_failed = true; failed = true; break; }
        accept = V.accept; chi2 = V.chi2; new_chi2 = V.new_chi2;
        if (accept) { S_old = S_new; nv_old = nv_new; cur ^= 1; }
      }
      if (A.rec && wg == 0 && threadIdx.x == 0 && n_rec < A.rec_cap) A.rec[(size_t)slot * A.rec_cap + n_rec] = svs_dense_lm_record{level, accept ? 1 : 0, chi2, new_chi2};
      ++n_rec;
      if (accept) {
        chi2 = new_chi2;
        double mx = -1;
        for (int q = 0; q < 6; ++q) mx = fmax(mx, fabs(s_x[q]));
        stop = mx <= 1e-10;
        if (threadIdx.x < 12) s_T[threadIdx.x] = s_Tn[threadIdx.x];
        if (threadIdx.x < 27) s_H[threadIdx.x] = s_out[threadIdx.x];
        __syncthreads();
      } else {
        stop = true;
      }
    }
    if (failed) break;
    if (solo) {
      __syncthreads();
      if (threadIdx.x < 12) __hip_atomic_store(G.bcast + (size_t)slot * 16 + threadIdx.x, s_T[threadIdx.x], __ATOMIC_RELAXED, __HIP_MEMORY_SCOPE_AGENT);
      asm volatile("s_waitcnt vmcnt(0)" ::: "memory");
      __syncthreads();
      if (threadIdx.x == 0) __hip_atomic_store(reinterpret_cast<unsigned *>(G.bcast + (size_t)slot * 16 + 12), 1u, __ATOMIC_RELAXED, __HIP_MEMORY_SCOPE_AGENT);
    }
  }
  __syncthreads();
  if (wg != 0) return;
  if (failed) { if (threadIdx.x == 0 && passes_out) passes_out[slot] = -1; return; }
  if (threadIdx.x < 12) T_io[(size_t)slot * 12 + threadIdx.x] = s_T[threadIdx.x];
  if (threadIdx.x == 0 && passes_out) passes_out[slot] = passes;
  if (threadIdx.x == 0 && A.n_rec) A.n_rec[slot] = n_rec;
  if (A.T_jac && threadIdx.x < 36) A.T_jac[(size_t)slot * 36 + threadIdx.x] = s_Tj[threadIdx.x / 12][threadIdx.x % 12];
  if (threadIdx.x == 0 && G.seq_stats && n_exact) {
    atomicAdd(G.seq_stats, n_exact);
    if (g_seq_sh.fell_back) atomicAdd(G.seq_stats + 1, 1u);
  }
}

struct TrkState {
  double S_old; float chi2, seq_old;
  int work16;
  int level, it, cur, passes, n_rec, nv_old, seq_old_ok, phase;
  unsigned n_exact;
};
__shared__ TrkState g_ts;
__shared__ double g_sT[12], g_sTn[12], g_sx[6], g_sH[27], g_sTj[3][12];
__device__ __noinline__ void track_solve_call() { track_solve(g_sH, g_sT, g_sTn, g_sx); }
struct TrkPark { TrkState ts; double T[12], H[27], Tj[36]; };
struct TrackCont { TrkPark *park; int *list; unsigned *count; int K; int slots; };
constexpr int CONT_MAX_NWG = 8;
template <bool U8SRC, bool MULTI>
__device__ __forceinline__ void track_batch_stream(const TrackArgs &A, double *__restrict__ T_io, int *__restrict__ passes_out, const TrackMulti &G, const TrackCont &C,
                                                   const int slot, const int wg, const int nwg) {
  constexpr int TM = MULTI ? 2 : 1;
  const int tid = threadIdx.x;
  __shared__ bool s_failed;
  float *const tb0 = G.terms ? G.terms + (size_t)slot * 2 * G.terms_b : nullptr;
  auto set_level = [&](int level) { g_pa.L = stream_level<U8SRC>(A, level, slot); g_pa.wg = wg; g_pa.nwg = nwg; };
  auto enter_level = [&](int level) {
    set_level(level);
    g_pa.t_buf = tb0;
    g_ts.level = level; g_ts.phase = 0; g_ts.cur = 0; g_ts.it = 0;
  };
  for (int i = tid; i < 256; i += TRK_THREADS) g_iplut[i] = (float)((1. / 255.) * i);
  if (tid == 0) { g_seq_sh.fell_back = 0; s_failed = false; }
  int sweep = 0;
  unsigned n_decisions = 0, n_old_sums = 0;
  if constexpr (!MULTI) {
    if (tid < 12) { const double v = T_io[(size_t)slot * 12 + tid]; g_sT[tid] = v; g_pa.T[tid] = v; }
    if (tid == 0) {
      g_ts.passes = 0; g_ts.n_rec = 0; g_ts.n_exact = 0; g_ts.work16 = 0;
      enter_level(2);
    }
    __syncthreads();
  } else {
    const TrkPark &P = C.park[slot];
    if (tid == 0) { g_ts = P.ts; if (wg != 0) g_ts.n_exact = 0; }
    if (tid < 12) g_sT[tid] = P.T[tid];
    if (tid >= 64 && tid < 64 + 27) g_sH[tid - 64] = P.H[tid - 64];
    if (tid >= 128 && tid < 128 + 36) g_sTj[(tid - 128) / 12][(tid - 128) % 12] = P.Tj[tid - 128];
    __syncthreads();
    if (tid == 0) set_level(g_ts.level);
    __syncthreads();
  }
  auto all_workgroups = [&]() {
    if (nwg == 1) return;
    sum_workgroups(G, slot, G.part + ((size_t)slot * 2 + (sweep & 1)) * CONT_MAX_NWG * 32, wg, nwg, sweep, s_failed);
  };
  bool failed = false, parked = false;
  bool resume = MULTI;
#pragma nounroll
  for (;;) {
    bool level_done = false;
    int level;
    if (!resume) {
      track_pass_from_lds<U8SRC, TM>();
      if constexpr (MULTI) { all_workgroups(); if (s_failed) { failed = true; break; } }
      level = g_ts.level;
      const int phase = g_ts.phase, cur = g_ts.cur, n_rec = g_ts.n_rec;
      const int n_lvl = (A.lv[level].cam.w / 4) * (A.lv[level].cam.h / 4);
      if (phase == 0) {
        const double S = g_s_out[27];
        const float chi2 = (float)S;
        __syncthreads();
        if (tid < 27) g_sH[tid] = g_s_out[tid];
        if (tid == 0) {
          g_ts.S_old = S; g_ts.nv_old = (int)g_s_out[NSUM]; g_ts.chi2 = chi2; g_ts.seq_old_ok = 0; g_ts.seq_old = 0.f;
          ++g_ts.passes; ++g_ts.n_rec; g_ts.work16 += 16 >> (2 * level);
          if (A.rec && wg == 0 && n_rec < A.rec_cap) A.rec[(size_t)slot * A.rec_cap + n_rec] = svs_dense_lm_record{level, 2, chi2, chi2};
        }
      } else {
        const double S_old = g_ts.S_old, S_new = g_s_out[27];
        const int nv_old = g_ts.nv_old, nv_new = (int)g_s_out[NSUM];
        float seq_old = g_ts.seq_old;
        bool seq_old_ok = g_ts.seq_old_ok != 0;
        unsigned n_exact = 0;
        const TrkVerdict V = track_accept<MULTI>(G, slot, S_old, S_new, nv_old, nv_new, tb0, cur, n_lvl, true, wg, nwg, g_ts.chi2, seq_old, seq_old_ok, n_decisions, n_old_sums, n_exact);
        if (V.failed) { if (tid == 0) s_failed = true; failed = true; break; }
        const bool accept = V.accept;
        const float chi2 = V.chi2, new_chi2 = V.new_chi2;
        double mx = -1;
        for (int q = 0; q < 6; ++q) mx = fmax(mx, fabs(g_sx[q]));
        const int it = g_ts.it + 1;
        level_done = !accept || mx <= 1e-10 || it >= 15;
        __syncthreads();
        if (accept) {
          if (tid < 12) g_sT[tid] = g_sTn[tid];
          if (tid < 27) g_sH[tid] = g_s_out[tid];
        }
        if (tid == 0) {
          if (accept) { g_ts.S_old = S_new; g_ts.nv_old = nv_new; g_ts.cur = cur ^ 1; g_ts.chi2 = new_chi2; }
          g_ts.seq_old = seq_old; g_ts.seq_old_ok = seq_old_ok ? 1 : 0; g_ts.it = it; g_ts.n_exact += n_exact;
          ++g_ts.passes; ++g_ts.n_rec; g_ts.work16 += 16 >> (2 * level);
          if (A.rec && wg == 0 && n_rec < A.rec_cap) A.rec[(size_t)slot * A.rec_cap + n_rec] = svs_dense_lm_record{level, accept ? 1 : 0, chi2, new_chi2};
        }
        if constexpr (!MULTI) {
          if (!level_done && level == 0 && C.K >= 0 && it >= C.K) parked = true;
        }
      }
      __syncthreads();
      if (parked) break;
    } else {
      resume = false;
      level = g_ts.level;
    }
    if (level_done) {
      if (level == 0) break;
      if (tid == 0) enter_level(level - 1);
      if (tid >= 64 && tid < 76) g_pa.T[tid - 64] = g_sT[tid - 64];
    } else {
      if (tid >= 64 && tid < 76) g_sTj[level][tid - 64] = g_sT[tid - 64];
      if (tid < 64) track_solve_call();
      __syncthreads();
      if (tid < 12) g_pa.T[tid] = g_sTn[tid];
      if (tid == 12) { g_pa.t_buf = tb0 ? tb0 + (size_t)(g_ts.cur ^ 1) * G.terms_b : nullptr; g_ts.phase = 1; }
    }
    __syncthreads();
  }
  if constexpr (!MULTI) {
    if (parked) {
      TrkPark &P = C.park[slot];
      if (tid == 0) { P.ts = g_ts; C.list[atomicAdd(C.count, 1u)] = slot; }
      if (tid < 12) P.T[tid] = g_sT[tid];
      if (tid >= 64 && tid < 64 + 27) P.H[tid - 64] = g_sH[tid - 64];
      if (tid >= 128 && tid < 128 + 36) P.Tj[tid - 128] = g_sTj[(tid - 128) / 12][(tid - 128) % 12];
      return;
    }
  }
  if (wg != 0) return;
  if (failed) { if (tid == 0 && passes_out) passes_out[slot] = -1; return; }
  if (tid < 12) T_io[(size_t)slot * 12 + tid] = g_sT[tid];
  if (tid == 0 && passes_out) passes_out[slot] = g_ts.passes;
  if (tid == 0 && A.n_rec) A.n_rec[slot] = g_ts.n_rec;
  if (tid == 0 && G.work16) G.work16[slot] = g_ts.work16;
  if (A.T_jac && tid < 36) A.T_jac[(size_t)slot * 36 + tid] = g_sTj[tid / 12][tid % 12];
  if (tid == 0 && G.seq_stats && g_ts.n_exact) {
    atomicAdd(G.seq_stats, g_ts.n_exact);
    if (g_seq_sh.fell_back) atomicAdd(G.seq_stats + 1, 1u);
  }
}
template <bool U8SRC, bool BAL, int CONT>
__global__ __launch_bounds__(TRK_THREADS, 4) void dense_track_batch_kernel(TrackArgs A, double *__restrict__ T_io, int *__restrict__ passes_out, TrackMulti G, TrackCont C) {
  if constexpr (CONT == 0) {
    int slot = blockIdx.x;
    if constexpr (BAL) {
      const int e = G.map[blockIdx.x];
      if (e < 0) return;
      slot = e >> 4;
    }
    track_batch_stream<U8SRC, false>(A, T_io, passes_out, G, C, slot, 0, 1);
  } else {
    const int n_parked = (int)*C.count;
    for (int p = blockIdx.y; p < n_parked; p += gridDim.y) {
      track_batch_stream<U8SRC, true>(A, T_io, passes_out, G, C, C.list[p], blockIdx.x, CONT_MAX_NWG);
      __syncthreads();
    }
  }
}

template <bool U8SRC>
__global__ __launch_bounds__(256) void residual_image_cpu_sem_kernel(LevelArgs L, size_t cloud_b, size_t prev_b, size_t f_b, size_t c8_b,
                                                                     const double *__restrict__ Tarr, size_t T_b,
                                                                     float *__restrict__ rimg, size_t rimg_b) {
  const int slot = blockIdx.y;
  const int cw = L.cam.w / 4, ch = L.cam.h / 4;
  const int i = blockIdx.x * 256 + threadIdx.x;
  if (i >= cw * ch) return;
  L.cloud += slot * cloud_b; L.prev += slot * prev_b;
  if (U8SRC) L.cur8 += slot * c8_b; else L.cur += slot * f_b;
  double T[12];
#pragma unroll
  for (int k = 0; k < 12; ++k) T[k] = Tarr[(size_t)slot * T_b + k];
  const int u = i % cw, v = i / cw;
  const float4 c4 = reinterpret_cast<const float4 *>(L.cloud)[i];
  float4 o = make_float4(0.f, 1.f, 0.f, 1.f);
  if (c4.w > 0) {
    const double xp0 = c4.x, xp1 = c4.y, xp2 = c4.z;
    const double x = T[0] * xp0 + T[1] * xp1 + T[2] * xp2 + T[3];
    const double y = T[4] * xp0 + T[5] * xp1 + T[6] * xp2 + T[7];
    const double z = T[8] * xp0 + T[9] * xp1 + T[10] * xp2 + T[11];
    const float uvx = (float)(L.cam.f * (x / z) + L.cam.cx);
    const float uvy = (float)(L.cam.f * (y / z) + L.cam.cy);
    bool ok = fabsf(uvx) < 1e9f && fabsf(uvy) < 1e9f;
    const int ui = ok ? (int)uvx : 0, vi = ok ? (int)uvy : 0;
    ok = ok && (ui >= 2 && vi >= 2 && ui < L.cam.w - 2 && vi < L.cam.h - 2);
    o = make_float4(1.f, 0.f, 0.f, 1.f);
    if (ok) {
      const float ip = (float)((1. / 255.) * L.prev[(size_t)(v * 4) * L.pstride + u * 4]);
      float ic, gx, gy;
      if (U8SRC) taps_u8(L.cur8, L.c8stride, uvx, uvy, ic, gx, gy);
      else ic = interp32f(L.cur, L.fstride, uvx, uvy);
      float res = ip - ic;
      if (res > 0.1) res = 0.1;
      if (res < -0.1) res = -0.1;
      float g = 1 - 50.f * res * res;
      if (g < 0.f) g = 0.f;
      o = make_float4(g, g, g, 1.f);
    }
  }
  reinterpret_cast<float4 *>(rimg + slot * rimg_b)[i] = o;
}


}


static bool offsets_fit_24(const svs_cam &cam, int pstride, int c8stride) {
  const int lim = 1 << 24;
  return cam.w > 0 && cam.h > 0 && cam.w < lim && cam.h < lim && pstride >= 0 && pstride < lim && c8stride >= 0 && c8stride < lim;
}
static int ensure_scratch(svs_ctx *ctx, double **p, size_t count) {
  void *v = nullptr;
  const int rc = svs_ctx_scratch(ctx, count * sizeof(double), &v);
  *p = static_cast<double *>(v);
  return rc;
}


extern "C" int svs_dense_pass_cpu_sem(svs_ctx *ctx, const float *d_cloud, size_t cloud_bstride, const uint8_t *d_prev_u8,
                                      int pstride, size_t p_bstride, const float *d_cur, const float *d_dx,
                                      const float *d_dy, int fstride, size_t f_bstride, const svs_cam *cam,
                                      const double *d_T, int do_jac, svs_dense_sums *d_out, int batch) {
  SVS_REQUIRE(ctx, ctx && d_cloud && d_prev_u8 && d_cur && cam && d_T && d_out && batch >= 1);
  SVS_DEVICE(ctx);
  SVS_REQUIRE(ctx, !do_jac || (d_dx && d_dy));
  SVS_REQUIRE(ctx, cam->w % 4 == 0 && cam->h % 4 == 0);
  SVS_REQUIRE(ctx, offsets_fit_24(*cam, pstride, 0));
  LevelArgs L{d_cloud, d_prev_u8, d_cur, d_dx, d_dy, pstride, fstride, *cam, nullptr, 0};
  int n = (cam->w / 4) * (cam->h / 4);
  int nblocks = std::min(div_up(n, 256), 256);
  double *part = nullptr;
  int rc = ensure_scratch(ctx, &part, (size_t)batch * nblocks * (NSUM + 1));
  if (rc) return rc;
  if (do_jac)
    hipLaunchKernelGGL(dense_pass_cpu_sem_kernel<true>, dim3(nblocks, batch), dim3(256), 0, ctx->stream, L, cloud_bstride, p_bstride, f_bstride, d_T, part);
  else
    hipLaunchKernelGGL(dense_pass_cpu_sem_kernel<false>, dim3(nblocks, batch), dim3(256), 0, ctx->stream, L, cloud_bstride, p_bstride, f_bstride, d_T, part);
  SVS_LAUNCH_CHECK(ctx);
  hipLaunchKernelGGL(dense_finalize_kernel, dim3(batch), dim3(64), 0, ctx->stream, part, nblocks, d_out);
  SVS_LAUNCH_CHECK(ctx);
  return SVS_OK;
}

namespace {
constexpr int BAL_MAX_STREAMS = 4096;
constexpr int ASSIGN_THREADS = 1024;
__global__ __launch_bounds__(ASSIGN_THREADS) void trk_assign_kernel(const int *__restrict__ work16, int B, int *__restrict__ map) {
  __shared__ __attribute__((aligned(16))) int s_key[BAL_MAX_STREAMS];
  const int tid = threadIdx.x;
  const int Bp = (B + 3) & ~3;
  for (int b = tid; b < Bp; b += ASSIGN_THREADS) s_key[b] = b < B ? (work16[b] << 12) | (4095 - b) : INT_MIN;
  __syncthreads();
  for (int b = tid; b < B; b += ASSIGN_THREADS) {
    const int mine = s_key[b];
    int pos = 0;
    for (int k = 0; k < Bp; k += 4) {
      const int4 q = *reinterpret_cast<const int4 *>(s_key + k);
      pos += (q.x > mine) + (q.y > mine) + (q.z > mine) + (q.w > mine);
    }
    map[pos] = b << 4;
  }
}

static int cont_setup(svs_ctx *ctx, int batch, TrackMulti &G, TrackCont &C) {
  const size_t n_part = (size_t)batch * 2 * CONT_MAX_NWG * 32, n_bar = (size_t)batch, n_bc = (size_t)batch * 16, n_cnt = 2, n_list = (size_t)batch / 2 + 1;
  const size_t n_park = ((size_t)batch * sizeof(TrkPark) + 7) / 8;
  double *scr = nullptr;
  const int rc = ensure_scratch(ctx, &scr, n_part + n_bar + n_bc + n_cnt + n_list + n_park);
  if (rc) return rc;
  G.part = scr;
  G.bar = reinterpret_cast<unsigned *>(scr + n_part);
  G.fail_off = batch;
  G.bcast = scr + n_part + n_bar;
  C.count = reinterpret_cast<unsigned *>(scr + n_part + n_bar + n_bc);
  C.list = reinterpret_cast<int *>(scr + n_part + n_bar + n_bc + n_cnt);
  C.park = reinterpret_cast<TrkPark *>(scr + n_part + n_bar + n_bc + n_cnt + n_list);
  C.K = ctx->trk_split; C.slots = ctx->trk_cont_slots > 0 ? ctx->trk_cont_slots : 2 * ctx->n_cu;
  SVS_HIP(ctx, hipMemsetAsync(G.bar, 0, sizeof(double) * (n_bar + n_bc + n_cnt), ctx->stream));
  return SVS_OK;
}
#define TRK_ARGS(...) __VA_ARGS__
#define TRK_LAUNCH(u8src, K, TAIL, grid, ...)                                                                              \
  do {                                                                                                                     \
    if (u8src) hipLaunchKernelGGL((K<true, TRK_ARGS TAIL>), grid, dim3(TRK_THREADS), 0, ctx->stream, __VA_ARGS__);         \
    else hipLaunchKernelGGL((K<false, TRK_ARGS TAIL>), grid, dim3(TRK_THREADS), 0, ctx->stream, __VA_ARGS__);              \
  } while (0)
template <bool BAL>
static int launch_batch_tracker(svs_ctx *ctx, const TrackArgs &A, bool u8src, double *d_T_io, int32_t *d_passes_out, int batch, TrackMulti G) {
  TrackCont C{nullptr, nullptr, nullptr, -1, 0};
  if (ctx->trk_split > 0) { const int rc = cont_setup(ctx, batch, G, C); if (rc) return rc; }
  TRK_LAUNCH(u8src, dense_track_batch_kernel, (BAL, 0), dim3(batch), A, d_T_io, d_passes_out, G, C);
  SVS_LAUNCH_CHECK(ctx);
  if (C.K < 0) return SVS_OK;
  const int groups = std::max(1, std::min(batch, C.slots / CONT_MAX_NWG));
  SvsSpinScope gate(ctx);
  if (gate.rc) return gate.rc;
  TRK_LAUNCH(u8src, dense_track_batch_kernel, (false, 1), dim3(CONT_MAX_NWG, groups), A, d_T_io, d_passes_out, G, C);
  SVS_LAUNCH_CHECK(ctx);
  return gate.leave();
}
struct BalState { int *map, *work16; };
size_t bal_row_bytes(int batch) { return (sizeof(int) * (size_t)batch + 255) & ~(size_t)255; }
BalState bal_state(void *state, int batch) {
  char *p = static_cast<char *>(state);
  return BalState{reinterpret_cast<int *>(p), reinterpret_cast<int *>(p + bal_row_bytes(batch))};
}
int bal_assign(svs_ctx *ctx, const BalState &S, int batch) {
  hipLaunchKernelGGL(trk_assign_kernel, dim3(1), dim3(ASSIGN_THREADS), 0, ctx->stream, S.work16, batch, S.map);
  SVS_LAUNCH_CHECK(ctx);
  return SVS_OK;
}
int svs_dense_track_cpu_sem_balanced(svs_ctx *ctx, const TrackArgs &A, bool u8src, double *d_T_io, int32_t *d_passes_out, int batch, void *state, TrackMulti G) {
  const BalState S = bal_state(state, batch);
  G.map = S.map; G.work16 = S.work16;
  if (int rc = launch_batch_tracker<true>(ctx, A, u8src, d_T_io, d_passes_out, batch, G)) return rc;
  return bal_assign(ctx, S, batch);
}
}
const int *svs_dense_track_balance_order(svs_ctx *ctx, void *state, int batch) {
  return state && ctx->trk_balance ? bal_state(state, batch).map : nullptr;
}
size_t svs_dense_track_balance_bytes(int batch) { return 2 * bal_row_bytes(batch); }
int svs_dense_track_balance_init(svs_ctx *ctx, void *state, int batch) {
  SVS_REQUIRE(ctx, ctx && state && batch >= 1 && batch <= BAL_MAX_STREAMS);
  SVS_DEVICE(ctx);
  SVS_HIP(ctx, hipMemsetAsync(state, 0, svs_dense_track_balance_bytes(batch), ctx->stream));
  return bal_assign(ctx, bal_state(state, batch), batch);
}
extern "C" int svs_dense_track_cpu_sem(svs_ctx *ctx, const svs_dense_track_args *a, double *d_T_io, int32_t *d_passes_out,
                                       int batch) {
  return svs_dense_track_cpu_sem_work(ctx, a, d_T_io, d_passes_out, batch, nullptr);
}
int svs_dense_track_cpu_sem_work(svs_ctx *ctx, const svs_dense_track_args *a, double *d_T_io, int32_t *d_passes_out, int batch, void *d_bal_state) {
  SVS_REQUIRE(ctx, ctx && a && d_T_io && batch >= 1);
  SVS_DEVICE(ctx);
  TrackArgs A;
  const bool u8src = a->d_cur_u8[0] != nullptr;
  for (int l = 0; l < 3; ++l) {
    SVS_REQUIRE(ctx, a->d_cloud[l] && a->d_prev_u8[l]);
    SVS_REQUIRE(ctx, u8src ? a->d_cur_u8[l] != nullptr : (a->d_cur[l] && a->d_dx[l] && a->d_dy[l]));
    SVS_REQUIRE(ctx, a->cam_vec[l].w % 4 == 0 && a->cam_vec[l].h % 4 == 0);
    SVS_REQUIRE(ctx, offsets_fit_24(a->cam_vec[l], a->pstride[l], u8src ? a->c8stride[l] : 0));
    A.lv[l] = LevelArgs{a->d_cloud[l], a->d_prev_u8[l], a->d_cur[l], a->d_dx[l], a->d_dy[l], a->pstride[l], a->fstride[l], a->cam_vec[l],
                        a->d_cur_u8[l], a->c8stride[l]};
    A.cloud_b[l] = a->cloud_bstride[l]; A.prev_b[l] = a->p_bstride[l]; A.f_b[l] = a->f_bstride[l]; A.c8_b[l] = a->c8_bstride[l];
  }
  A.T_jac = a->d_T_jac_out;
  A.rec = a->d_record_out; A.rec_cap = a->d_record_out ? a->record_cap : 0; A.n_rec = a->d_n_record_out;
  SVS_REQUIRE(ctx, !a->d_record_out || a->record_cap > 0);
  int nwg = batch <= 16 ? 8 : (batch <= 32 ? 4 : 1);
  if (ctx->trk_nwg) nwg = ctx->trk_nwg;
  float *t_buf = nullptr; size_t t_b = 0;
  const bool seq_all = ctx->trk_seq_chi2 != 0, lazy = !seq_all && ctx->trk_lazy_chi2 != 0;
  float *terms = nullptr;
  if (seq_all || lazy) {
    if (seq_all) nwg = 1;
    t_b = (size_t)(a->cam_vec[0].w / 4) * (a->cam_vec[0].h / 4);
    if (lazy) t_b = ((t_b + 3) & ~(size_t)3) + 64;
    const size_t want = (size_t)batch * t_b * sizeof(float) * (lazy ? 2 : 1) + 256;
    if (ctx->seq_buf.bytes() < want) {
      if (ctx->seq_buf) SVS_HIP(ctx, hipStreamSynchronize(ctx->stream));
      SVS_HIP(ctx, ctx->seq_buf.reserve(want, want));
    }
    if (seq_all) t_buf = static_cast<float *>(ctx->seq_buf.get()); else terms = static_cast<float *>(ctx->seq_buf.get());
    if (!ctx->seq_stats) {
      SVS_HIP(ctx, ctx->seq_stats.alloc_bytes(256));
      SVS_HIP(ctx, hipMemsetAsync(ctx->seq_stats, 0, 256, ctx->stream));
    }
  }
  TrackMulti G{};
  G.terms = terms; G.terms_b = t_b; G.seq_stats = ctx->seq_stats; G.terms_only = ctx->trk_lazy_chi2 == 2;
  enum class Form { SeqChain, Latency, BigOrdered, Big, OnePerCu };
  const bool ordered = d_bal_state && ctx->trk_balance && batch >= 2 * ctx->n_cu && batch <= BAL_MAX_STREAMS && A.rec && A.n_rec;
  const bool big = (batch > ctx->n_cu && ctx->trk_regs != 1) || ctx->trk_regs == 2;
  const Form form = t_buf ? Form::SeqChain : nwg >= 2 ? Form::Latency : ordered ? Form::BigOrdered : big ? Form::Big : Form::OnePerCu;
  switch (form) {
    case Form::SeqChain:
      G.part = reinterpret_cast<double *>(t_buf); G.fail_off = (int)t_b;
      TRK_LAUNCH(u8src, dense_track_cpu_sem_kernel, (false, true), dim3(batch), A, d_T_io, d_passes_out, G);
      break;
    case Form::Latency: {
      double *scratch = nullptr;
      const size_t n_part = (size_t)batch * 2 * nwg * 64;
      const size_t n_clear = (n_part + (size_t)batch + (size_t)batch * 16 + 7) & ~(size_t)7;
      int rc = ensure_scratch(ctx, &scratch, n_clear);
      if (rc) return rc;
      G.part = scratch;
      G.bar = reinterpret_cast<unsigned *>(scratch + n_part);
      G.fail_off = batch;
      G.bcast = scratch + n_part + (size_t)batch;
      SVS_HIP(ctx, hipMemsetAsync(scratch, 0, sizeof(double) * n_clear, ctx->stream));
      SvsSpinScope gate(ctx, nwg * batch);
      if (gate.rc) return gate.rc;
      TRK_LAUNCH(u8src, dense_track_cpu_sem_kernel, (true), dim3(nwg, batch), A, d_T_io, d_passes_out, G);
      SVS_LAUNCH_CHECK(ctx);
      if (int grc = gate.leave()) return grc;
      break;
    }
    case Form::BigOrdered: return svs_dense_track_cpu_sem_balanced(ctx, A, u8src, d_T_io, d_passes_out, batch, d_bal_state, G);
    case Form::Big: return launch_batch_tracker<false>(ctx, A, u8src, d_T_io, d_passes_out, batch, G);
    case Form::OnePerCu:
      TRK_LAUNCH(u8src, dense_track_cpu_sem_kernel, (false), dim3(batch), A, d_T_io, d_passes_out, G);
      break;
  }
  SVS_LAUNCH_CHECK(ctx);
  return SVS_OK;
}

namespace {
template <int HOW>
__global__ __launch_bounds__(TRK_THREADS) void seq_sum_probe_kernel(const float *__restrict__ t, int n, size_t bstride, float *__restrict__ out, int *__restrict__ fell_back) {
  if (threadIdx.x == 0) g_seq_sh.fell_back = 0;
  __syncthreads();
  const float *row = t + (size_t)blockIdx.x * bstride;
  float v;
  if constexpr (HOW == 2) v = seq_chi2_f32(row, n); else v = exact_seq_sum_f32<HOW == 1>(row, n);
  if (threadIdx.x == 0) { out[blockIdx.x] = v; if (fell_back) fell_back[blockIdx.x] = HOW == 2 ? 1 : g_seq_sh.fell_back; }
}
}
extern "C" int svs_dense_seq_sum_f32(svs_ctx *ctx, const float *d_terms, int n, size_t bstride, int batch, int how, float *d_out, int32_t *d_fell_back) {
  SVS_REQUIRE(ctx, ctx && d_terms && d_out && n >= 0 && batch >= 1 && how >= 0 && how <= 2);
  SVS_DEVICE(ctx);
  if (how == 0) hipLaunchKernelGGL(seq_sum_probe_kernel<0>, dim3(batch), dim3(TRK_THREADS), 0, ctx->stream, d_terms, n, bstride, d_out, d_fell_back);
  else if (how == 1) hipLaunchKernelGGL(seq_sum_probe_kernel<1>, dim3(batch), dim3(TRK_THREADS), 0, ctx->stream, d_terms, n, bstride, d_out, d_fell_back);
  else hipLaunchKernelGGL(seq_sum_probe_kernel<2>, dim3(batch), dim3(TRK_THREADS), 0, ctx->stream, d_terms, n, bstride, d_out, d_fell_back);
  SVS_LAUNCH_CHECK(ctx);
  return SVS_OK;
}

extern "C" int svs_dense_residual_image_cpu_sem(svs_ctx *ctx, const float *d_cloud, size_t cloud_bstride, const uint8_t *d_prev_u8,
                                                int pstride, size_t p_bstride, const float *d_cur, int fstride, size_t f_bstride,
                                                const uint8_t *d_cur_u8, int c8stride, size_t c8_bstride, const svs_cam *cam,
                                                const double *d_T, size_t T_bstride, float *d_res_img4, size_t res_bstride, int batch) {
  SVS_REQUIRE(ctx, ctx && d_cloud && d_prev_u8 && (d_cur || d_cur_u8) && cam && d_T && d_res_img4 && batch >= 1);
  SVS_DEVICE(ctx);
  SVS_REQUIRE(ctx, cam->w % 4 == 0 && cam->h % 4 == 0);
  SVS_REQUIRE(ctx, offsets_fit_24(*cam, pstride, d_cur_u8 ? c8stride : 0));
  LevelArgs L{d_cloud, d_prev_u8, d_cur, nullptr, nullptr, pstride, fstride, *cam, d_cur_u8, c8stride};
  const int n = (cam->w / 4) * (cam->h / 4);
  if (d_cur_u8)
    hipLaunchKernelGGL(residual_image_cpu_sem_kernel<true>, dim3(div_up(n, 256), batch), dim3(256), 0, ctx->stream, L, cloud_bstride, p_bstride,
                       f_bstride, c8_bstride, d_T, T_bstride, d_res_img4, res_bstride);
  else
    hipLaunchKernelGGL(residual_image_cpu_sem_kernel<false>, dim3(div_up(n, 256), batch), dim3(256), 0, ctx->stream, L, cloud_bstride, p_bstride,
                       f_bstride, c8_bstride, d_T, T_bstride, d_res_img4, res_bstride);
  SVS_LAUNCH_CHECK(ctx);
  return SVS_OK;
}
```

scavislam_amd/csrc/seqsum.h:

```cpp
#pragma once
#include <stdint.h>
#include <string.h>

#if defined(__HIPCC__)
#define SVS_SEQ_HD __host__ __device__ __forceinline__
#else
#define SVS_SEQ_HD static inline
#endif

struct SvsSeqMap { int32_t d0, dd; };

SVS_SEQ_HD uint32_t svs_seq_bits(float f) { uint32_t u; memcpy(&u, &f, 4); return u; }
SVS_SEQ_HD float svs_seq_float(uint32_t u) { float f; memcpy(&f, &u, 4); return f; }

constexpr int32_t SVS_SEQ_CARRY = 1 << 24;

SVS_SEQ_HD bool svs_seq_add_term(SvsSeqMap &m, uint32_t tb, int eb) {
  if (tb == 0) return false;
  int et = (int)(tb >> 23);
  uint32_t mt = tb & 0x7fffffu;
  if (et == 0) et = 1; else mt |= 0x800000u;
  const int shift = eb - et;
  if (shift > 24) return false;
  if (shift < 0) { m.d0 = SVS_SEQ_CARRY; m.dd = 0; return false; }
  const uint32_t q = mt >> shift;
  const uint32_t rem = mt & ((1u << shift) - 1u);
  const uint32_t half = (1u << shift) >> 1;
  const bool tie = shift > 0 && rem == half;
  if (!tie) {
    const int32_t inc = (int32_t)q + (rem > half ? 1 : 0);
    m.d0 = m.d0 + inc < SVS_SEQ_CARRY ? m.d0 + inc : SVS_SEQ_CARRY;
    return false;
  }
  const int32_t c0 = (m.d0 + (int32_t)q) & 1, c1 = (1 + m.d0 + m.dd + (int32_t)q) & 1;
  const int32_t n0 = m.d0 + (int32_t)q + c0;
  m.d0 = n0 < SVS_SEQ_CARRY ? n0 : SVS_SEQ_CARRY;
  m.dd += c1 - c0;
  return true;
}
SVS_SEQ_HD bool svs_seq_add_term_fast(SvsSeqMap &m, float t, int eb) {
  const float base = svs_seq_float((uint32_t)eb << 23), half_ulp = svs_seq_float((uint32_t)(eb - 24) << 23);
  const float s_ = base + t, d = s_ - base, r = t - d;
  const int32_t inc = (int32_t)(svs_seq_bits(s_) - ((uint32_t)eb << 23));
  const bool tie = (r < 0 ? -r : r) == half_ulp;
  if (!tie) { m.d0 += inc; return false; }
  const int32_t sg = r > 0 ? 1 : -1;
  const int32_t par0 = m.d0 & 1, par1 = (1 + m.d0 + m.dd) & 1;
  const int32_t n0 = m.d0 + inc + (par0 ? sg : 0), n1 = m.d0 + m.dd + inc + (par1 ? sg : 0);
  m.d0 = n0; m.dd = n1 - n0;
  return true;
}
SVS_SEQ_HD SvsSeqMap svs_seq_compose(const SvsSeqMap &f, const SvsSeqMap &g) {
  const int32_t f0 = f.d0, f1 = f.d0 + f.dd;
  const int32_t g0 = g.d0, g1 = g.d0 + g.dd;
  const int32_t r0 = f0 + ((f0 & 1) ? g1 : g0);
  const int32_t r1 = f1 + (((1 + f1) & 1) ? g1 : g0);
  SvsSeqMap r;
  r.d0 = r0 < SVS_SEQ_CARRY ? r0 : SVS_SEQ_CARRY;
  r.dd = r1 - r0;
  if (r.dd > 1 || r.dd < -1) r.dd = 0;
  return r;
}
SVS_SEQ_HD bool svs_seq_safe(double P_s, double P_e, int c_s, int c_e, int *eb) {
  if (!(c_s >= 1) || !(P_s > 0.0) || c_e > 300000) return false;
  const double u = 5.9604644775390625e-08;
  const double lo = P_s * (1.0 - (1.0001 * c_s * u + 1e-12)), hi = P_e * (1.0 + (1.0001 * c_e * u + 1e-12));
  uint64_t a, b;
  memcpy(&a, &lo, 8); memcpy(&b, &hi, 8);
  const int ea = (int)((a >> 52) & 0x7ff) - 1023, ebb = (int)((b >> 52) & 0x7ff) - 1023;
  if (ea != ebb || ea < -100 || ea > 100) return false;
  *eb = ea + 127;
  return true;
}
SVS_SEQ_HD bool svs_seq_apply(float *acc, const SvsSeqMap &m, int eb) {
  const uint32_t bits = svs_seq_bits(*acc);
  if ((int)(bits >> 23) != eb) return false;
  const uint32_t A = (bits & 0x7fffffu) | 0x800000u;
  const int64_t A2 = (int64_t)A + ((A & 1u) ? (int64_t)m.d0 + m.dd : (int64_t)m.d0);
  if (A2 >= (int64_t)SVS_SEQ_CARRY || m.d0 >= SVS_SEQ_CARRY) return false;
  *acc = svs_seq_float(((uint32_t)eb << 23) | ((uint32_t)A2 & 0x7fffffu));
  return true;
}
```

Before: 218,900 frames/s.

## Parallelize exact sequential-sum rescue and overlap old/new sums with speculative solve

Reworks the exact sequential float sum used in dense tracking's accept test. Unsafe runs are now split into quads, each with its own safe-exponent map, so the serial wave walk only replays short unsafe stretches instead of whole runs. The old and new chi2 sums are computed together in one pass, with one wave walking each. A spare wave speculatively solves the next LM step while they run. This adds LDS usage, more barriers and considerable complexity in exchange for less serialized work per LM iteration.

```diff
diff --git a/include/scavislam_hip.h b/include/scavislam_hip.h
--- a/include/scavislam_hip.h
+++ b/include/scavislam_hip.h
@@ -220,6 +220,8 @@
 int svs_dense_track_cpu_sem(svs_ctx *ctx, const svs_dense_track_args *a, double *d_T_io,
                             int32_t *d_passes_out, int batch);
 int svs_dense_seq_sum_f32(svs_ctx *ctx, const float *d_terms, int n, size_t bstride, int batch, int how, float *d_out, int32_t *d_fell_back);
+int svs_dense_seq_sum_pair_f32(svs_ctx *ctx, const float *d_terms_a, const float *d_terms_b, int n, size_t bstride, int batch, int how, float *d_out_a, float *d_out_b,
+                               int32_t *d_fell_back);
 int svs_dense_residual_image_cpu_sem(svs_ctx *ctx, const float *d_cloud, size_t cloud_bstride,
                                      const uint8_t *d_prev_u8, int pstride, size_t p_bstride,
                                      const float *d_cur, int fstride, size_t f_bstride,
diff --git a/scavislam_amd/capi.py b/scavislam_amd/capi.py
--- a/scavislam_amd/capi.py
+++ b/scavislam_amd/capi.py
@@ -115,6 +115,7 @@
                                C.c_void_p, C.c_void_p, C.c_void_p, C.c_int, C.c_size_t, C.POINTER(Cam),
                                C.c_void_p, C.c_int, C.c_void_p, C.c_int],
     "svs_dense_seq_sum_f32": [C.c_void_p, C.c_void_p, C.c_int, C.c_size_t, C.c_int, C.c_int, C.c_void_p, C.c_void_p],
+    "svs_dense_seq_sum_pair_f32": [C.c_void_p, C.c_void_p, C.c_void_p, C.c_int, C.c_size_t, C.c_int, C.c_int, C.c_void_p, C.c_void_p, C.c_void_p],
     "svs_dense_track_cpu_sem": [C.c_void_p, C.POINTER(DenseTrackArgs), C.c_void_p, C.c_void_p, C.c_int],
     "svs_dense_residual_image_cpu_sem": [C.c_void_p, C.c_void_p, C.c_size_t, C.c_void_p, C.c_int, C.c_size_t,
                                          C.c_void_p, C.c_int, C.c_size_t, C.c_void_p, C.c_int, C.c_size_t,
diff --git a/scavislam_amd/csrc/dense.hip b/scavislam_amd/csrc/dense.hip
--- a/scavislam_amd/csrc/dense.hip
+++ b/scavislam_amd/csrc/dense.hip
@@ -360,15 +360,23 @@
 
 constexpr int SEQ_Q = TRK_THREADS >= 512 ? 10 : 13;
 constexpr int SEQ_RUN_MAX = 4 * SEQ_Q;
-constexpr int SEQ_STAGE_FLOATS = 48 * SEQ_RUN_MAX;
+constexpr int SEQ_SLOTS = 24;
 struct SeqShared {
   SvsSeqMap pref[TRK_THREADS];
   unsigned char eb[TRK_THREADS];
   short slot[TRK_THREADS];
+  unsigned short stretch[TRK_THREADS];
   unsigned long long unsafe[TRK_THREADS / 64];
   double wave_P[TRK_THREADS / 64];
-  int wave_c[TRK_THREADS / 64], wave_u[TRK_THREADS / 64];
-  float stage[SEQ_STAGE_FLOATS];
+  int wave_c[TRK_THREADS / 64];
+  unsigned nslots;
+  SvsSeqGroup wave_tail[TRK_THREADS / 64];
+  SvsSeqGroup last;
+  double run_P[SEQ_SLOTS];
+  int run_c[SEQ_SLOTS];
+  unsigned char qe[SEQ_SLOTS * SEQ_Q];
+  SvsSeqMap qm[SEQ_SLOTS * SEQ_Q];
+  float stage[SEQ_SLOTS * SEQ_RUN_MAX];
   float result;
   int fell_back;
 };
@@ -403,19 +411,12 @@
     for (int q = 0; q < SEQ_Q; ++q) v[q] = q < nq ? *reinterpret_cast<svs_gptr_f4>(p + 4 * q) : svs_f4{0.f, 0.f, 0.f, 0.f};
   }
 }
-__shared__ SeqShared g_seq_sh;
+__device__ __forceinline__ SvsSeqGroup seq_group_up(const SvsSeqGroup &g, int d) {
+  return SvsSeqGroup{SvsSeqMap{__shfl_up(g.m.d0, d, 64), __shfl_up(g.m.dd, d, 64)}, __shfl_up(g.eb, d, 64)};
+}
 template <bool COH>
-__device__ __noinline__ float exact_seq_sum_f32(const float *t_flat, int n) {
-  SeqShared &sh = g_seq_sh;
-  svs_gptr_f32 t = (svs_gptr_f32)t_flat;
+__device__ __forceinline__ void seq_prepare_runs(SeqShared &sh, svs_gptr_f32 t, int n, int S) {
   const int tid = threadIdx.x, lane = tid & 63, wave = tid >> 6;
-  const int S = max(4, (div_up(n, TRK_THREADS) + 3) & ~3);
-  if (S > SEQ_RUN_MAX) {
-    __syncthreads();
-    if (wave == 0) { const float v = seq_sum_f32<COH, svs_gptr_f32>(t, n); if (lane == 0) { sh.result = v; sh.fell_back = 1; } }
-    __syncthreads();
-    return sh.result;
-  }
   const int nq = S / 4;
   const int j0 = min(n, tid * S), j1 = min(n, j0 + S);
   const bool empty = j0 >= j1;
@@ -439,7 +440,6 @@
     const int oc = __shfl_up(cincl, d, 64);
     if (lane >= d) { incl += o; cincl += oc; }
   }
-  __syncthreads();
   if (lane == 63) { sh.wave_P[wave] = incl; sh.wave_c[wave] = cincl; }
   __syncthreads();
   double base = 0;
@@ -450,19 +450,11 @@
   const double P_s = base + (lane ? excl : 0.0), P_e = P_s + ps;
   const int c_s = cbase + (lane ? cexcl : 0), c_e = c_s + cnt;
   int eb = 0;
-  bool safe = empty || svs_seq_safe(P_s, P_e, c_s, c_e, &eb);
+  const bool safe = empty || svs_seq_safe(P_s, P_e, c_s, c_e, &eb);
+  int slot = -1;
+  if (!safe) { slot = (int)atomicAdd(&sh.nslots, 1u); if (slot >= SEQ_SLOTS) slot = -1; }
+  sh.slot[tid] = (short)slot;
   sh.eb[tid] = (safe && !empty) ? (unsigned char)eb : (unsigned char)0;
-  __syncthreads();
-  if (safe && !empty && tid > 0) { const int pe = sh.eb[tid - 1]; if (pe != 0 && pe != eb) safe = false; }
-  const unsigned long long um = __ballot(!safe);
-  if (lane == 0) { sh.unsafe[wave] = um; sh.wave_u[wave] = __popcll(um); }
-  __syncthreads();
-  int ubase = 0;
-  for (int w = 0; w < wave; ++w) ubase += sh.wave_u[w];
-  const int uidx = ubase + __popcll(um & ((1ull << lane) - 1ull));
-  const int slot = (!safe && (uidx + 1) * S <= SEQ_STAGE_FLOATS) ? uidx : -1;
-  sh.slot[tid] = (short)slot;
-  if (!safe) sh.eb[tid] = 0;
   SvsSeqMap m{0, 0};
   if (safe) {
 #pragma unroll
@@ -472,75 +464,190 @@
   } else if (slot >= 0) {
 #pragma unroll
     for (int q = 0; q < SEQ_Q; ++q)
-      if (q < nq) *reinterpret_cast<svs_f4 *>(&sh.stage[slot * S + 4 * q]) = v[q];
-  }
-  bool flag = !safe || lane == 0;
+      if (q < nq) *reinterpret_cast<svs_f4 *>(&sh.stage[slot * SEQ_RUN_MAX + 4 * q]) = v[q];
+    sh.run_P[slot] = P_s; sh.run_c[slot] = c_s;
+  }
+  sh.pref[tid] = m;
+}
+__device__ __forceinline__ void seq_prepare_groups(SeqShared &sh, int n, int S) {
+  const int tid = threadIdx.x, lane = tid & 63, wave = uni_i32(tid >> 6);
+  const int nq = S / 4;
+  const int len = max(0, min(S, n - tid * S)), nqr = (len + 3) >> 2;
+  {
+    const int nslots = min((int)sh.nslots, SEQ_SLOTS);
+    if (tid < nslots * nq) {
+      const int r = tid / nq, q = tid - r * nq;
+      int e;
+      SvsSeqMap m;
+      svs_seq_quad<SEQ_Q>(&sh.stage[r * SEQ_RUN_MAX], q, sh.run_P[r], sh.run_c[r], &e, &m);
+      sh.qe[r * SEQ_Q + q] = (unsigned char)e;
+      sh.qm[r * SEQ_Q + q] = m;
+    }
+  }
+  const int slot = sh.slot[tid], eb_run = sh.eb[tid];
+  const SvsSeqMap m_run = sh.pref[tid];
+  __syncthreads();
+  int pe = 0;
+  if (tid > 0) {
+    const int sp = sh.slot[tid - 1], lq = (min(S, n - (tid - 1) * S) + 3) >> 2;
+    pe = sp >= 0 ? sh.qe[sp * SEQ_Q + lq - 1] : sh.eb[tid - 1];
+  }
+  SvsSeqGroup head{m_run, eb_run}, tail{SvsSeqMap{0, 0}, 0};
+  int fu = nqr, lu = -1;
+  if (slot >= 0) svs_seq_run_parts<SEQ_Q>(&sh.qe[slot * SEQ_Q], &sh.qm[slot * SEQ_Q], nqr, pe, &head, &tail, &fu, &lu);
+  else if (nqr > 0 && (eb_run == 0 || (pe != 0 && pe != eb_run))) { head = tail; fu = 0; lu = nqr - 1; }
+  const bool unsafe = fu < nqr;
+  const unsigned long long um = __ballot(unsafe);
+  if (lane == 0) sh.unsafe[wave] = um;
+  SvsSeqGroup Z = unsafe ? tail : head;
+  bool flag = unsafe;
 #pragma unroll
   for (int d = 1; d < 64; d <<= 1) {
-    const int o0 = __shfl_up(m.d0, d, 64), o1 = __shfl_up(m.dd, d, 64), of = __shfl_up((int)flag, d, 64);
-    if (lane >= d && !flag) { m = svs_seq_compose(SvsSeqMap{o0, o1}, m); flag = of != 0; }
-  }
-  sh.pref[tid] = m;
-  __syncthreads();
-  if (wave == 0) {
-    float acc = 0.f;
-    bool ok = true;
-    const int nseg = div_up(n, S);
-    for (int chunk = 0; chunk * 64 < nseg && ok; ++chunk) {
-      const int limit = min(64, nseg - chunk * 64);
-      const unsigned long long mask = sh.unsafe[chunk];
-      const SvsSeqMap my = sh.pref[chunk * 64 + lane];
-      const int my_eb = sh.eb[chunk * 64 + lane], my_sl = sh.slot[chunk * 64 + lane];
-      auto run_terms = [&](int idx) {
-        const int seg = chunk * 64 + idx, sj0 = seg * S, len = min(S, n - sj0), sl = __builtin_amdgcn_readlane(my_sl, idx);
-        float x = sh.stage[(sl >= 0 && lane < len) ? sl * S + lane : 0];
-        if (sl < 0) x = seq_term_load<COH, svs_gptr_f32>(t + sj0 + (lane < len ? lane : 0));
-        return lane < len ? x : 0.f;
-      };
-      unsigned long long m = limit < 64 ? mask & ((1ull << limit) - 1ull) : mask;
-      float x_next = m ? run_terms((int)__builtin_ctzll(m)) : 0.f;
-      int pos = 0;
-      while (ok) {
-        const int nxt = m ? (int)__builtin_ctzll(m) : limit;
-        if (nxt > pos) {
-          const SvsSeqMap g{__builtin_amdgcn_readlane(my.d0, nxt - 1), __builtin_amdgcn_readlane(my.dd, nxt - 1)};
-          ok = svs_seq_apply(&acc, g, __builtin_amdgcn_readlane(my_eb, nxt - 1));
-        }
-        if (nxt >= limit || !ok) break;
-        m &= m - 1ull;
-        const float x = x_next;
-        if (m) x_next = run_terms((int)__builtin_ctzll(m));
-#pragma unroll
-        for (int l = 0; l < SEQ_RUN_MAX; ++l) acc = acc + __builtin_bit_cast(float, __builtin_amdgcn_readlane(__builtin_bit_cast(int, x), l));
-        pos = nxt + 1;
+    const SvsSeqGroup o = seq_group_up(Z, d);
+    const int of = __shfl_up((int)flag, d, 64);
+    if (lane >= d && !flag) { Z = svs_seq_join(o, Z); flag = of != 0; }
+  }
+  if (lane == 63) sh.wave_tail[wave] = Z;
+  __syncthreads();
+  SvsSeqGroup carry{SvsSeqMap{0, 0}, 0};
+#pragma unroll
+  for (int w = 0; w < TRK_THREADS / 64 - 1; ++w) {
+    const SvsSeqGroup wt = sh.wave_tail[w];
+    const bool wu = sh.unsafe[w] != 0;
+    if (w < wave) carry = wu ? wt : svs_seq_join(carry, wt);
+  }
+  if ((um & (lane == 63 ? ~0ull : (2ull << lane) - 1ull)) == 0) Z = svs_seq_join(carry, Z);
+  SvsSeqGroup prev = seq_group_up(Z, 1);
+  if (lane == 0) prev = carry;
+  if (unsafe) {
+    const SvsSeqGroup front = svs_seq_join(prev, head);
+    const int slen = min(4 * (lu + 1), len) - 4 * fu;
+    sh.pref[tid] = front.m;
+    sh.eb[tid] = (unsigned char)front.eb;
+    sh.stretch[tid] = (unsigned short)(4 * fu | slen << 8);
+  }
+  if (tid == TRK_THREADS - 1) sh.last = Z;
+}
+template <bool COH>
+__device__ __forceinline__ float seq_walk(SeqShared &sh, svs_gptr_f32 t, int n, int S, bool *fell_back) {
+  const int lane = threadIdx.x & 63;
+  float acc = 0.f;
+  bool ok = true;
+  const int nseg = div_up(n, S);
+  for (int chunk = 0; chunk * 64 < nseg && ok; ++chunk) {
+    const unsigned long long m_v = sh.unsafe[chunk];
+    unsigned long long m = ((unsigned long long)(unsigned)uni_i32((int)(m_v >> 32)) << 32) | (unsigned)uni_i32((int)m_v);
+    if (!m) continue;
+    const SvsSeqMap my = sh.pref[chunk * 64 + lane];
+    const int my_eb = sh.eb[chunk * 64 + lane], my_sl = sh.slot[chunk * 64 + lane], my_st = sh.stretch[chunk * 64 + lane];
+    auto stretch_terms = [&](int idx) {
+      const int sl = __builtin_amdgcn_readlane(my_sl, idx), st = __builtin_amdgcn_readlane(my_st, idx);
+      const int off = st & 255, len = st >> 8, sj0 = (chunk * 64 + idx) * S + off;
+      float x = sh.stage[(sl >= 0 && lane < len) ? sl * SEQ_RUN_MAX + off + lane : 0];
+      if (sl < 0) x = seq_term_load<COH, svs_gptr_f32>(t + sj0 + (lane < len ? lane : 0));
+      return lane < len ? x : 0.f;
+    };
+    float x_next = stretch_terms((int)__builtin_ctzll(m));
+    while (m) {
+      const int idx = (int)__builtin_ctzll(m);
+      m &= m - 1ull;
+      const int e = __builtin_amdgcn_readlane(my_eb, idx), len = __builtin_amdgcn_readlane(my_st, idx) >> 8;
+      if (e) {
+        const SvsSeqMap g{__builtin_amdgcn_readlane(my.d0, idx), __builtin_amdgcn_readlane(my.dd, idx)};
+        ok = svs_seq_apply(&acc, g, e);
+        if (!ok) break;
       }
-    }
-    if (!ok) acc = seq_sum_f32<COH, svs_gptr_f32>(t, n);
-    if (lane == 0) { sh.result = acc; if (!ok) sh.fell_back = 1; }
-  }
-  __syncthreads();
-  return sh.result;
+      const float x = x_next;
+      if (m) x_next = stretch_terms((int)__builtin_ctzll(m));
+#pragma unroll
+      for (int q = 0; q < SEQ_Q; ++q) {
+        if (4 * q >= len) break;
+#pragma unroll
+        for (int c = 0; c < 4; ++c) acc = acc + __builtin_bit_cast(float, __builtin_amdgcn_readlane(__builtin_bit_cast(int, x), 4 * q + c));
+      }
+    }
+  }
+  if (ok) { const SvsSeqGroup g = sh.last; if (g.eb) ok = svs_seq_apply(&acc, g.m, g.eb); }
+  if (!ok) acc = seq_sum_f32<COH, svs_gptr_f32>(t, n);
+  *fell_back = !ok;
+  return acc;
+}
+__shared__ SeqShared g_seq_sh[2];
+__device__ __noinline__ void track_solve_call(int spec);
+__device__ __forceinline__ int seq_run_len(int n) { return max(4, (div_up(n, TRK_THREADS) + 3) & ~3); }
+__shared__ const float *g_seq_t[2];
+__shared__ int g_seq_n;
+template <bool COH>
+__device__ __noinline__ void seq_prepare_runs_call(int s) {
+  const int n = g_seq_n;
+  seq_prepare_runs<COH>(g_seq_sh[s], (svs_gptr_f32)g_seq_t[s], n, seq_run_len(n));
+}
+__device__ __noinline__ void seq_prepare_groups_call(int s_in) {
+  const int n = uni_i32(g_seq_n), s = uni_i32(s_in);
+  seq_prepare_groups(g_seq_sh[s], n, seq_run_len(n));
+}
+template <bool COH>
+__device__ __noinline__ void seq_walk_call() {
+  const int lane = threadIdx.x & 63, wave = uni_i32((int)(threadIdx.x >> 6));
+  svs_gptr_f32 t = (svs_gptr_f32)uni_ptr(g_seq_t[wave]);
+  const int n = uni_i32(g_seq_n);
+  const int S = seq_run_len(n);
+  bool fb = true;
+  const float v = S > SEQ_RUN_MAX ? seq_sum_f32<COH, svs_gptr_f32>(t, n) : seq_walk<COH>(g_seq_sh[wave], t, n, S, &fb);
+  if (lane == 0) { g_seq_sh[wave].result = v; if (fb) g_seq_sh[0].fell_back = 1; }
+}
+template <bool COH, bool SPEC = false>
+__device__ __forceinline__ void exact_seq_sums(const float *t0, const float *t1, int n, int ns) {
+  const bool par = ns > 0 && seq_run_len(n) <= SEQ_RUN_MAX;
+  if (threadIdx.x == 0) { g_seq_t[0] = t0; g_seq_t[1] = t1; g_seq_n = n; g_seq_sh[0].nslots = 0; g_seq_sh[1].nslots = 0; }
+  __syncthreads();
+  if (par) {
+    seq_prepare_runs_call<COH>(0);
+    if (ns > 1) seq_prepare_runs_call<COH>(1);
+    __syncthreads();
+    seq_prepare_groups_call(0);
+    if (ns > 1) seq_prepare_groups_call(1);
+  }
+  __syncthreads();
+  const int wave = threadIdx.x >> 6;
+  if (wave < ns) seq_walk_call<COH>();
+  else if (SPEC && wave == 2) track_solve_call(1);
+  __syncthreads();
+}
+template <bool COH, bool SPEC = false>
+__device__ __forceinline__ float exact_seq_sum_f32(const float *t, int n) {
+  exact_seq_sums<COH, SPEC>(t, t, n, 1);
+  return g_seq_sh[0].result;
 }
 
 struct NearSums { float seq_old, seq_new; bool failed; };
-template <bool COH>
+template <bool COH, bool SPEC>
 __device__ __forceinline__ NearSums shared_near_sums(const float *t_old, const float *t_new, int n, int wg, int nwg, bool need_old, float seq_old_in, unsigned n_dec, unsigned n_old,
                                                      double *bc, unsigned *fail_word, unsigned &n_exact) {
   __shared__ unsigned long long s_words[2];
   __shared__ int s_nf;
   NearSums R{seq_old_in, 0.f, false};
   if (nwg <= 1) {
-    if (need_old) { R.seq_old = exact_seq_sum_f32<COH>(t_old, n); ++n_exact; }
-    R.seq_new = exact_seq_sum_f32<COH>(t_new, n); ++n_exact;
+    if (need_old) {
+      exact_seq_sums<COH, SPEC>(t_new, t_old, n, 2);
+      R.seq_new = g_seq_sh[0].result; R.seq_old = g_seq_sh[1].result; n_exact += 2;
+    } else {
+      R.seq_new = exact_seq_sum_f32<COH, SPEC>(t_new, n); ++n_exact;
+    }
     return R;
   }
   unsigned long long *w_new = reinterpret_cast<unsigned long long *>(bc + 13), *w_old = reinterpret_cast<unsigned long long *>(bc + 15);
-  if (wg == 0) {
-    R.seq_new = exact_seq_sum_f32<COH>(t_new, n); ++n_exact;
-    if (threadIdx.x == 0) __hip_atomic_store(w_new, ((unsigned long long)n_dec << 32) | (unsigned long long)__float_as_uint(R.seq_new), __ATOMIC_RELAXED, __HIP_MEMORY_SCOPE_AGENT);
-  } else if (wg == 1 && need_old) {
-    R.seq_old = exact_seq_sum_f32<COH>(t_old, n); ++n_exact;
-    if (threadIdx.x == 0) __hip_atomic_store(w_old, ((unsigned long long)n_old << 32) | (unsigned long long)__float_as_uint(R.seq_old), __ATOMIC_RELAXED, __HIP_MEMORY_SCOPE_AGENT);
+  {
+    const bool forms = wg == 0 || (wg == 1 && need_old);
+    const float *const tt = wg == 0 ? t_new : t_old;
+    exact_seq_sums<COH, SPEC>(tt, tt, n, forms ? 1 : 0);
+    if (forms) {
+      const float v = g_seq_sh[0].result;
+      ++n_exact;
+      if (wg == 0) R.seq_new = v; else R.seq_old = v;
+      if (threadIdx.x == 0)
+        __hip_atomic_store(wg == 0 ? w_new : w_old, ((unsigned long long)(wg == 0 ? n_dec : n_old) << 32) | (unsigned long long)__float_as_uint(v), __ATOMIC_RELAXED, __HIP_MEMORY_SCOPE_AGENT);
+    }
   }
   if (threadIdx.x == 0) {
     int nf = 0;
@@ -586,8 +693,8 @@
   else { L.cur += slot * A.f_b[level]; L.dx += slot * A.f_b[level]; L.dy += slot * A.f_b[level]; }
   return L;
 }
-__device__ __forceinline__ void track_solve(const double (&sH)[27], const double (&sT)[12], double (&sTn)[12], double (&sx)[6]) {
-  const int lane = threadIdx.x;
+__device__ __forceinline__ void track_solve(const double *sH, const double *sT, double *sTn, double *sx) {
+  const int lane = threadIdx.x & 63;
   double col[6], x[6], Tc[12], Tn[12];
 #pragma unroll
   for (int r = 0; r < 6; ++r) {
@@ -632,19 +739,20 @@
   }
   __syncthreads();
 }
-struct TrkVerdict { bool accept, failed; float chi2, new_chi2; };
-template <bool MULTI>
+struct TrkVerdict { bool accept, failed; float chi2, new_chi2; bool solved; };
+template <bool MULTI, bool SPEC = false>
 __device__ __forceinline__ TrkVerdict track_accept(const TrackMulti &G, int slot, double S_old, double S_new, int nv_old, int nv_new, const float *tb0, int cur,
                                                    int n_lvl, bool counted, int wg, int nwg, float chi2, float &seq_old, bool &seq_old_ok,
                                                    unsigned &n_decisions, unsigned &n_old_sums, unsigned &n_exact) {
-  TrkVerdict V{false, false, chi2, 0.f};
+  TrkVerdict V{false, false, chi2, 0.f, false};
   const double gam = 1.0001 * (double)max(nv_old, nv_new) * 5.9604644775390625e-08 + 1e-12;
   const bool near = tb0 && !G.terms_only && !(fabs(S_old - S_new) > gam * (S_old + S_new));
   if (near) {
     if (counted) { ++n_decisions; if (!seq_old_ok) ++n_old_sums; }
-    const NearSums ns = shared_near_sums<MULTI>(tb0 + (size_t)cur * G.terms_b, tb0 + (size_t)(cur ^ 1) * G.terms_b, n_lvl, wg, nwg, !seq_old_ok, seq_old, n_decisions, n_old_sums,
+    const NearSums ns = shared_near_sums<MULTI, SPEC>(tb0 + (size_t)cur * G.terms_b, tb0 + (size_t)(cur ^ 1) * G.terms_b, n_lvl, wg, nwg, !seq_old_ok, seq_old, n_decisions, n_old_sums,
                                                 MULTI ? G.bcast + (size_t)slot * 16 : nullptr, MULTI ? G.bar + G.fail_off + slot : nullptr, n_exact);
     if (ns.failed) { V.failed = true; return V; }
+    V.solved = SPEC;
     seq_old = ns.seq_old;
     seq_old_ok = true;
     V.chi2 = seq_old; V.new_chi2 = ns.seq_new;
@@ -664,7 +772,7 @@
   float (&s_iplut)[256] = g_iplut;
   __shared__ double s_T[12], s_Tn[12], s_x[6], s_H[27], s_Tj[3][12];
   __shared__ bool s_failed;
-  if (threadIdx.x == 0) { s_failed = false; if (!SEQ) g_seq_sh.fell_back = 0; }
+  if (threadIdx.x == 0) { s_failed = false; if (!SEQ) g_seq_sh[0].fell_back = 0; }
   constexpr int TM = SEQ ? 1 : (MULTI ? 2 : 1);
   unsigned n_exact = 0, n_decisions = 0, n_old_sums = 0;
   const int slot = MULTI ? blockIdx.y : blockIdx.x, wg = MULTI ? blockIdx.x : 0;
@@ -802,7 +910,7 @@
   if (A.T_jac && threadIdx.x < 36) A.T_jac[(size_t)slot * 36 + threadIdx.x] = s_Tj[threadIdx.x / 12][threadIdx.x % 12];
   if (threadIdx.x == 0 && G.seq_stats && n_exact) {
     atomicAdd(G.seq_stats, n_exact);
-    if (g_seq_sh.fell_back) atomicAdd(G.seq_stats + 1, 1u);
+    if (g_seq_sh[0].fell_back) atomicAdd(G.seq_stats + 1, 1u);
   }
 }
 
@@ -813,8 +921,13 @@
   unsigned n_exact;
 };
 __shared__ TrkState g_ts;
-__shared__ double g_sT[12], g_sTn[12], g_sx[6], g_sH[27], g_sTj[3][12];
-__device__ __noinline__ void track_solve_call() { track_solve(g_sH, g_sT, g_sTn, g_sx); }
+__shared__ int g_solved;
+__shared__ double g_sT[12], g_sTn[12], g_sx[6], g_sH[27], g_sTj[3][12], g_sTn2[12], g_sx2[6];
+__device__ __noinline__ void track_solve_call(int spec) {
+  const double *H = spec ? g_s_out : g_sH, *T = spec ? g_sTn : g_sT;
+  double *Tn = spec ? g_sTn2 : g_sTn, *x = spec ? g_sx2 : g_sx;
+  track_solve(H, T, Tn, x);
+}
 struct TrkPark { TrkState ts; double T[12], H[27], Tj[36]; };
 struct TrackCont { TrkPark *park; int *list; unsigned *count; int K; int slots; };
 constexpr int CONT_MAX_NWG = 8;
@@ -832,7 +945,7 @@
     g_ts.level = level; g_ts.phase = 0; g_ts.cur = 0; g_ts.it = 0;
   };
   for (int i = tid; i < 256; i += TRK_THREADS) g_iplut[i] = (float)((1. / 255.) * i);
-  if (tid == 0) { g_seq_sh.fell_back = 0; s_failed = false; }
+  if (tid == 0) { g_seq_sh[0].fell_back = 0; s_failed = false; }
   int sweep = 0;
   unsigned n_decisions = 0, n_old_sums = 0;
   if constexpr (!MULTI) {
@@ -861,6 +974,7 @@
 #pragma nounroll
   for (;;) {
     bool level_done = false;
+    if (tid == 0) g_solved = 0;
     int level;
     if (!resume) {
       track_pass_from_lds<U8SRC, TM>();
@@ -884,7 +998,7 @@
         float seq_old = g_ts.seq_old;
         bool seq_old_ok = g_ts.seq_old_ok != 0;
         unsigned n_exact = 0;
-        const TrkVerdict V = track_accept<MULTI>(G, slot, S_old, S_new, nv_old, nv_new, tb0, cur, n_lvl, true, wg, nwg, g_ts.chi2, seq_old, seq_old_ok, n_decisions, n_old_sums, n_exact);
+        const TrkVerdict V = track_accept<MULTI, !MULTI>(G, slot, S_old, S_new, nv_old, nv_new, tb0, cur, n_lvl, true, wg, nwg, g_ts.chi2, seq_old, seq_old_ok, n_decisions, n_old_sums, n_exact);
         if (V.failed) { if (tid == 0) s_failed = true; failed = true; break; }
         const bool accept = V.accept;
         const float chi2 = V.chi2, new_chi2 = V.new_chi2;
@@ -893,9 +1007,12 @@
         const int it = g_ts.it + 1;
         level_done = !accept || mx <= 1e-10 || it >= 15;
         __syncthreads();
+        const bool solved = V.solved && accept && !level_done;
+        if (tid == 0 && solved) g_solved = 1;
         if (accept) {
-          if (tid < 12) g_sT[tid] = g_sTn[tid];
+          if (tid < 12) { g_sT[tid] = g_sTn[tid]; if (solved) g_sTn[tid] = g_sTn2[tid]; }
           if (tid < 27) g_sH[tid] = g_s_out[tid];
+          if (solved && tid >= 32 && tid < 38) g_sx[tid - 32] = g_sx2[tid - 32];
         }
         if (tid == 0) {
           if (accept) { g_ts.S_old = S_new; g_ts.nv_old = nv_new; g_ts.cur = cur ^ 1; g_ts.chi2 = new_chi2; }
@@ -919,7 +1036,7 @@
       if (tid >= 64 && tid < 76) g_pa.T[tid - 64] = g_sT[tid - 64];
     } else {
       if (tid >= 64 && tid < 76) g_sTj[level][tid - 64] = g_sT[tid - 64];
-      if (tid < 64) track_solve_call();
+      if (!g_solved && tid < 64) track_solve_call(0);
       __syncthreads();
       if (tid < 12) g_pa.T[tid] = g_sTn[tid];
       if (tid == 12) { g_pa.t_buf = tb0 ? tb0 + (size_t)(g_ts.cur ^ 1) * G.terms_b : nullptr; g_ts.phase = 1; }
@@ -945,7 +1062,7 @@
   if (A.T_jac && tid < 36) A.T_jac[(size_t)slot * 36 + tid] = g_sTj[tid / 12][tid % 12];
   if (tid == 0 && G.seq_stats && g_ts.n_exact) {
     atomicAdd(G.seq_stats, g_ts.n_exact);
-    if (g_seq_sh.fell_back) atomicAdd(G.seq_stats + 1, 1u);
+    if (g_seq_sh[0].fell_back) atomicAdd(G.seq_stats + 1, 1u);
   }
 }
 template <bool U8SRC, bool BAL, int CONT>
@@ -1219,12 +1336,20 @@
 namespace {
 template <int HOW>
 __global__ __launch_bounds__(TRK_THREADS) void seq_sum_probe_kernel(const float *__restrict__ t, int n, size_t bstride, float *__restrict__ out, int *__restrict__ fell_back) {
-  if (threadIdx.x == 0) g_seq_sh.fell_back = 0;
+  if (threadIdx.x == 0) g_seq_sh[0].fell_back = 0;
   __syncthreads();
   const float *row = t + (size_t)blockIdx.x * bstride;
   float v;
   if constexpr (HOW == 2) v = seq_chi2_f32(row, n); else v = exact_seq_sum_f32<HOW == 1>(row, n);
-  if (threadIdx.x == 0) { out[blockIdx.x] = v; if (fell_back) fell_back[blockIdx.x] = HOW == 2 ? 1 : g_seq_sh.fell_back; }
+  if (threadIdx.x == 0) { out[blockIdx.x] = v; if (fell_back) fell_back[blockIdx.x] = HOW == 2 ? 1 : g_seq_sh[0].fell_back; }
+}
+template <int HOW>
+__global__ __launch_bounds__(TRK_THREADS) void seq_sum_probe_pair_kernel(const float *__restrict__ ta, const float *__restrict__ tb, int n, size_t bstride, float *__restrict__ out_a,
+                                                                         float *__restrict__ out_b, int *__restrict__ fell_back) {
+  if (threadIdx.x == 0) g_seq_sh[0].fell_back = 0;
+  __syncthreads();
+  exact_seq_sums<HOW == 1>(ta + (size_t)blockIdx.x * bstride, tb + (size_t)blockIdx.x * bstride, n, 2);
+  if (threadIdx.x == 0) { out_a[blockIdx.x] = g_seq_sh[0].result; out_b[blockIdx.x] = g_seq_sh[1].result; if (fell_back) fell_back[blockIdx.x] = g_seq_sh[0].fell_back; }
 }
 }
 extern "C" int svs_dense_seq_sum_f32(svs_ctx *ctx, const float *d_terms, int n, size_t bstride, int batch, int how, float *d_out, int32_t *d_fell_back) {
@@ -1233,6 +1358,16 @@
   if (how == 0) hipLaunchKernelGGL(seq_sum_probe_kernel<0>, dim3(batch), dim3(TRK_THREADS), 0, ctx->stream, d_terms, n, bstride, d_out, d_fell_back);
   else if (how == 1) hipLaunchKernelGGL(seq_sum_probe_kernel<1>, dim3(batch), dim3(TRK_THREADS), 0, ctx->stream, d_terms, n, bstride, d_out, d_fell_back);
   else hipLaunchKernelGGL(seq_sum_probe_kernel<2>, dim3(batch), dim3(TRK_THREADS), 0, ctx->stream, d_terms, n, bstride, d_out, d_fell_back);
+  SVS_LAUNCH_CHECK(ctx);
+  return SVS_OK;
+}
+
+extern "C" int svs_dense_seq_sum_pair_f32(svs_ctx *ctx, const float *d_terms_a, const float *d_terms_b, int n, size_t bstride, int batch, int how, float *d_out_a, float *d_out_b,
+                                          int32_t *d_fell_back) {
+  SVS_REQUIRE(ctx, ctx && d_terms_a && d_terms_b && d_out_a && d_out_b && n >= 0 && batch >= 1 && how >= 0 && how <= 1);
+  SVS_DEVICE(ctx);
+  if (how == 0) hipLaunchKernelGGL(seq_sum_probe_pair_kernel<0>, dim3(batch), dim3(TRK_THREADS), 0, ctx->stream, d_terms_a, d_terms_b, n, bstride, d_out_a, d_out_b, d_fell_back);
+  else hipLaunchKernelGGL(seq_sum_probe_pair_kernel<1>, dim3(batch), dim3(TRK_THREADS), 0, ctx->stream, d_terms_a, d_terms_b, n, bstride, d_out_a, d_out_b, d_fell_back);
   SVS_LAUNCH_CHECK(ctx);
   return SVS_OK;
 }
diff --git a/scavislam_amd/csrc/seqsum.h b/scavislam_amd/csrc/seqsum.h
--- a/scavislam_amd/csrc/seqsum.h
+++ b/scavislam_amd/csrc/seqsum.h
@@ -4,9 +4,12 @@
 
 #if defined(__HIPCC__)
 #define SVS_SEQ_HD __host__ __device__ __forceinline__
+#define SVS_SEQ_UNROLL _Pragma("unroll")
 #else
 #define SVS_SEQ_HD static inline
+#define SVS_SEQ_UNROLL
 #endif
+
 
 struct SvsSeqMap { int32_t d0, dd; };
 
@@ -81,3 +84,57 @@
   *acc = svs_seq_float(((uint32_t)eb << 23) | ((uint32_t)A2 & 0x7fffffu));
   return true;
 }
+
+
+struct SvsSeqGroup { SvsSeqMap m; int32_t eb; };
+SVS_SEQ_HD SvsSeqGroup svs_seq_join(const SvsSeqGroup &f, const SvsSeqGroup &g) {
+  SvsSeqGroup r;
+  r.m = svs_seq_compose(f.m, g.m);
+  r.eb = f.eb ? f.eb : g.eb;
+  if (f.eb && g.eb && f.eb != g.eb) { r.m.d0 = SVS_SEQ_CARRY; r.m.dd = 0; }
+  return r;
+}
+template <int NQ>
+SVS_SEQ_HD void svs_seq_quad(const float *run, int q, double P_s, int c_s, int *e, SvsSeqMap *m) {
+  double P = P_s;
+  int c = c_s;
+  float x[4] = {0.f, 0.f, 0.f, 0.f};
+  SVS_SEQ_UNROLL
+  for (int j = 0; j < NQ; ++j) {
+    if (j > q) continue;
+    float y[4];
+    for (int k = 0; k < 4; ++k) y[k] = run[4 * j + k];
+    if (j < q) { for (int k = 0; k < 4; ++k) { P += (double)y[k]; c += y[k] != 0.f ? 1 : 0; } }
+    else { for (int k = 0; k < 4; ++k) x[k] = y[k]; }
+  }
+  double Pn = P;
+  int cn = c;
+  for (int k = 0; k < 4; ++k) { Pn += (double)x[k]; cn += x[k] != 0.f ? 1 : 0; }
+  int eb = 0;
+  if (!svs_seq_safe(P, Pn, c, cn, &eb)) eb = 0;
+  SvsSeqMap mm{0, 0};
+  if (eb != 0)
+    for (int k = 0; k < 4; ++k) svs_seq_add_term_fast(mm, x[k], eb);
+  *e = eb; *m = mm;
+}
+template <int NQ>
+SVS_SEQ_HD void svs_seq_run_parts(const unsigned char *qe, const SvsSeqMap *qm, int nqr, int pe, SvsSeqGroup *head, SvsSeqGroup *tail, int *fu, int *lu) {
+  int f = nqr, l = -1, prev = pe;
+  SvsSeqGroup g[NQ];
+  SVS_SEQ_UNROLL
+  for (int q = 0; q < NQ; ++q) { g[q].m = qm[q]; g[q].eb = qe[q]; }
+  SVS_SEQ_UNROLL
+  for (int q = 0; q < NQ; ++q) {
+    if (q >= nqr) continue;
+    const int e = g[q].eb;
+    if (e == 0 || (prev != 0 && prev != e)) { if (f == nqr) f = q; l = q; }
+    prev = e;
+  }
+  SvsSeqGroup h{{0, 0}, 0}, t{{0, 0}, 0};
+  SVS_SEQ_UNROLL
+  for (int q = 0; q < NQ; ++q) {
+    if (q < f) h = svs_seq_join(h, g[q]);
+    else if (q > l && q < nqr) t = svs_seq_join(t, g[q]);
+  }
+  *head = h; *tail = t; *fu = f; *lu = l;
+}
```

Result: no change. 220,400 frames/s, median of 6 (+0.7%).
